# l646773422/h264-lab

Measured on AMD Instinct MI355X. Metric: 1080p macroblocks/sec, higher is better.
Workload: dtype u8

## Files before the change

### h264-lab_amd/csrc/h264e_host.c

```c
#include <stdio.h>
#include <stdlib.h>
#include <string.h>
#include <time.h>
#include <sched.h>
#include <pthread.h>
#include "../../include/h264e_mi355x.h"
#include "../../include/h264e_hip.h"

#define MAGIC 0x4D493335u
#define SLICE_P 0
#define SLICE_I 2

static int g_device = -1;
static __thread char g_host_err[256];

static int imin(int a, int b) { return a < b ? a : b; }
static int imax(int a, int b) { return a > b ? a : b; }

const char *H264E_last_error(void) { return g_host_err[0] ? g_host_err : h264e_hip_last_error(); }
void H264E_set_device(int device) { g_device = device; }
int H264E_device_count(void) { return h264e_hip_device_count(); }

static int pick_device(void)
{
// ... 723 lines not shown
        return H264E_STATUS_BAD_FRAME_TYPE;

    qp = rc_frame_start(&e->rc, e->param.gop, e->seq.nmb, e->param.vbv_size_bytes, opt->desired_frame_bytes,
                        e->run_param.qp_min, e->run_param.qp_max, key);

    memset(&task, 0, sizeof(task));
    task.active = 1; task.frame_index = 0;
    task.slice_type = key ? SLICE_I : SLICE_P;
    task.qp = qp; task.speed = opt->encode_speed;
    task.nslices = e->slices > 1 ? imin(e->slices, e->seq.nmby) : 1;
    slice_header_bits(&e->seq, key, e->frame_num, e->next_idr_pic_id, qp, e->pic_init_qp,
                      (opt->encode_speed == 8 || opt->encode_speed == 10), task.nslices, &task.hdr_nal, &task.hdr_bits, &task.hdr_nbits);
    build_qdat(task.qdat, qp, !key);

    memset(&res, 0, sizeof(res));
    den = e->denoise && opt->encode_speed < 2;
    if (den)
    {
        if (put_frame(m->pool, in, dev, win) || h264e_hip_denoise_frames(m->pool, 0, 1, !e->den_started)) return H264E_STATUS_BAD_ARGUMENT;
        e->den_started = 1;
        task.denoised = 1;
    }
    e->frames_in++;
    if (e->param.vbv_size_bytes && !key && e->rc.vbv_bits - opt->desired_frame_bytes*8 > e->param.vbv_size_bytes*8)
    {
        uint8_t rb[32];
        hbits_t b;
        size_t w;
        memset(&b, 0, sizeof(b));
        b.buf = rb;
        hb_put(&b, 8, (uint32_t)task.hdr_nal);
        hb_ue(&b, 0);
        hb_put(&b, task.hdr_nbits > 32 ? task.hdr_nbits - 32 : 0, (uint32_t)(task.hdr_nbits > 32 ? task.hdr_bits >> 32 : 0));
        hb_put(&b, task.hdr_nbits > 32 ? 32 : task.hdr_nbits, (uint32_t)task.hdr_bits);
        hb_ue(&b, (uint32_t)e->seq.nmb);
        hb_put(&b, 1, 1);
        if (b.n) hb_put(&b, 8 - b.n, 0);
        if (out_pos + 2*b.pos + 8 > cap) { snprintf(g_host_err, sizeof(g_host_err), "coded frame does not fit the scratch blob"); return H264E_STATUS_BAD_ARGUMENT; }
        w = nal_emit(out + out_pos, rb, b.pos);
        if (opt->nalu_callback) opt->nalu_callback(out + out_pos + 4, (int)(w - 4), opt->nalu_callback_token);
        out_pos += w;
        res.all_skipped = 1;
        if (!den && put_frame(m->pool, in, dev, win)) return H264E_STATUS_BAD_ARGUMENT;
    } else
    {
    if (!den && put_frame(m->pool, in, dev, win)) return H264E_STATUS_BAD_ARGUMENT;
    if (frame_exact(m->pool, &task, e->seq.nmbx, e->seq.nmby, e->clusters) || h264e_hip_stream_done(m->pool, 0, &res) != 1) return H264E_STATUS_BAD_ARGUMENT;
    {
        const uint8_t *nals = frame_nals(m->pool, 0, &res, m->rbsp, m->rbsp_cap);
        size_t w;
        if (!nals) return H264E_STATUS_BAD_ARGUMENT;
        w = emit_slices(out + out_pos, cap - out_pos, nals, &res, opt->nalu_callback, opt->nalu_callback_token);
        if (!w)
        {
            snprintf(g_host_err, sizeof(g_host_err), "coded frame does not fit the scratch blob");
            return H264E_STATUS_BAD_ARGUMENT;
        }
        out_pos += w;
    }
    }

    if (task.nslices == 1 || res.all_skipped) e->parent_all_skipped = res.all_skipped;
    rc_frame_end(&e->rc, e->seq.nmb, e->param.vbv_size_bytes, opt->desired_frame_bytes, (int)out_pos, key, e->parent_all_skipped);

    if (!e->param.const_input_flag && in)
    {
        int c, y;
        const uint8_t *s = m->recon;
        if (h264e_hip_read_recon(m->pool, 0, m->recon)) return H264E_STATUS_BAD_ARGUMENT;
        for (c = 0; c < 3; c++)
        {
            int w = e->seq.w >> (c ? 1 : 0), h = e->seq.h >> (c ? 1 : 0);
            for (y = 0; y < h; y++) memcpy(in->yuv[c] + (size_t)y*in->stride[c], s + (size_t)y*w, (size_t)w);
            s += (size_t)w*h;
        }
    }
    if (++e->frame_num >= e->param.gop && e->param.gop && e->run_param.frame_type == H264E_FRAME_TYPE_DEFAULT) e->frame_num = 0;
    e->have_recon = 1;
    *coded_data = out;
    *sizeof_coded_data = (int)out_pos;
    return H264E_STATUS_SUCCESS;
}

int H264E_encode(H264E_persist_t *p, H264E_scratch_t *scratch, const H264E_run_param_t *opt, H264E_io_yuv_t *in,
                 unsigned char **coded_data, int *sizeof_coded_data)
{
    return encode_frame(p, scratch, opt, in, NULL, NULL, coded_data, sizeof_coded_data);
}

int H264E_encode_device(H264E_persist_t *p, H264E_scratch_t *scratch, const H264E_run_param_t *opt, const H264E_dev_frame_t *frame,
                        unsigned char **coded_data, int *sizeof_coded_data)
{
    return encode_frame(p, scratch, opt, NULL, frame, NULL, coded_data, sizeof_coded_data);
}

int H264E_encode_device_scaled(H264E_persist_t *p, H264E_scratch_t *scratch, const H264E_run_param_t *opt, const H264E_dev_frame_t *frame,
                               const H264E_dev_window_t *win, unsigned char **coded_data, int *sizeof_coded_data)
{
    if (!frame || !win)
    {
        snprintf(g_host_err, sizeof(g_host_err), "H264E_encode_device_scaled: null %s", frame ? "window" : "frame");
        return H264E_STATUS_BAD_ARGUMENT;
    }
    return encode_frame(p, scratch, opt, NULL, frame, win, coded_data, sizeof_coded_data);
}

int H264E_read_recon_device(H264E_persist_t *p, const H264E_dev_frame_t *dst)
{
    henc_t *e = (henc_t *)p;
    impl_t mm;
    g_host_err[0] = 0;
    if (!impl_of(e, &mm)) return H264E_STATUS_BAD_ARGUMENT;
    if (!dst) { snprintf(g_host_err, sizeof(g_host_err), "H264E_read_recon_device: null destination"); return H264E_STATUS_BAD_ARGUMENT; }
    if (!e->have_recon)
    {
        snprintf(g_host_err, sizeof(g_host_err), "H264E_read_recon_device: no frame has been encoded yet");
        return H264E_STATUS_BAD_ARGUMENT;
    }
    return h264e_hip_egress_last(mm.pool, 0, dst->format, (void *const *)dst->plane, dst->stride, dst->pixel_bytes, dst->producer_stream) ? H264E_STATUS_BAD_ARGUMENT
                                                                                                                                     : H264E_STATUS_SUCCESS;
}

int H264E_read_quality(H264E_persist_t *p, uint64_t ssd[3], double ssim[3])
{
    henc_t *e = (henc_t *)p;
    impl_t mm;
    g_host_err[0] = 0;
    if (!impl_of(e, &mm)) return H264E_STATUS_BAD_ARGUMENT;
    if (!ssd && !ssim) { snprintf(g_host_err, sizeof(g_host_err), "H264E_read_quality: both outputs are NULL"); return H264E_STATUS_BAD_ARGUMENT; }
    if (!e->have_recon)
    {
        snprintf(g_host_err, sizeof(g_host_err), "H264E_read_quality: no frame has been encoded yet");
        return H264E_STATUS_BAD_ARGUMENT;
    }
    return h264e_hip_quality_last(mm.pool, 0, ssd, ssim) ? H264E_STATUS_BAD_ARGUMENT : H264E_STATUS_SUCCESS;
}

int H264E_ssim_planes(int device, const void *a, int a_stride, const void *b, int b_stride, int width, int height, double *ssim)
{
    h264e_hip_pool_t *pool = NULL;
    int rc;
    g_host_err[0] = 0;
    if (h264e_hip_pool_create(&pool, device < 0 ? pick_device() : device, 16, 16, 1, 1)) return -1;
    rc = h264e_hip_ssim_planes(pool, a, a_stride, b, b_stride, width, height, ssim);
    h264e_hip_pool_destroy(pool);
    return rc;
}

void *H264E_dev_malloc(int device, size_t bytes) { g_host_err[0] = 0; return h264e_hip_dev_malloc(device, bytes); }
void H264E_dev_free(void *p) { h264e_hip_dev_free(p); }
int H264E_dev_memcpy(void *dst, const void *src, size_t bytes, int to_device) { g_host_err[0] = 0; return h264e_hip_dev_memcpy(dst, src, bytes, to_device); }


#define CLIP_KEEP_MAX 8
typedef struct { int done, ring_lo, entries; } clip_pass_t;
struct H264E_clip_tag
{
    H264E_clip_param_t par;
    seq_t seq;
    int nframes, ring;
    int resident;
    int time_input;
    double input_ms;
    long long input_frames;
    h264e_hip_pool_t *pool;
    int next;
    int avail;
    int pending_avail;
    void (*idle_hook)(void *token); void *idle_token;
    int32_t state[2];
    int first_dev;
    int first_row;
    int32_t after[2]; int have_after;
    int narrow;
    int narrow_ok;
    int wide_until, wide_hold;
    int launch_base, launch_frames;
    int stopped_before;
    long long far_acc; int far_frames;
    int rc_on;
    rc_t rcs; int rc_frame, rc_qp;
    int rc_last_bytes[2];
    h264e_hip_mbrec_t **rec_store;
    int32_t (*used_store)[2];
    int32_t **permb_store;
    uint64_t *ssd_out;
    double *ssim_out;
    int recon_floor;
    int32_t *traj;
    uint8_t *big; size_t big_cap;
    h264e_hip_task_t *tasks;
    int32_t (*used)[2];
    clip_pass_t sc, la, den;
    int denoise, den_motion;
    struct clip_sched { uint8_t key, idr; int frame_num; } *sched;
    int *forced, nforced;
    int all_key;
    int scenecut;
    uint32_t *sc_hist;
    int *sc_dist; uint8_t *sc_cut;
    double sc_kernel_ms; long long sc_frames;
    uint8_t *qp_sched;
    int qp_explicit;
    int la_kbps, la_window, la_qmin, la_qmax;
    uint64_t *la_rec;
    int *la_bits;
    int la_planned, la_closed;
    uint64_t la_k[2];
    long long la_debt;
    double la_kernel_ms; long long la_frames;
    int la_search, la_any;
    int keep_on;
    int nkeep;
    struct clip_keep { int frame, rows, qp, nslices, speed, denoised; } keep[CLIP_KEEP_MAX];
};

static void clip_keep_drop(H264E_clip_t *c, int from)
{
    int i, k = 0;
    for (i = 0; i < c->nkeep; i++) if (c->keep[i].frame < from) c->keep[k++] = c->keep[i];
    c->nkeep = k;
}


static int clip_pass_pending(const H264E_clip_t *c, const clip_pass_t *p, const char *pass, int limit)
{
    if (limit - p->done > c->resident) { snprintf(g_host_err, sizeof(g_host_err), "%s: frames %d..%d do not fit the input ring", pass, p->done, limit - 1); return -1; }
    return imax(limit - p->done, 0);
}

static void clip_pass_made(clip_pass_t *p, int a, int limit)
{
    p->done = limit;
    p->ring_lo = imax(imin(p->ring_lo, a), limit - p->entries);
}

static int clip_pass_resident(const clip_pass_t *p, int frame, const char *who, const char *what)
{
    const int hi = p->done, lo = imin(p->ring_lo, hi);
    if (frame >= lo && frame < hi) return 1;
    if (lo < hi) snprintf(g_host_err, sizeof(g_host_err), "%s: frame %d has no %s on the device (frames %d..%d have)", who, frame, what, lo, hi - 1);
    else snprintf(g_host_err, sizeof(g_host_err), "%s: frame %d has no %s on the device (no frame has)", who, frame, what);
    return 0;
}

static void clip_inputs_replaced(H264E_clip_t *c, int first)
{
    if (first < c->sc.done) c->sc.done = first;
    if (first < c->la.done) c->la.done = first;
    if (first < c->den.done) c->den.done = first;
    clip_keep_drop(c, first);
}

static int clip_pass_predecessor_gone(const clip_pass_t *p, int first, const char *made, const char *kept, const char *ring)
{
    if (first <= 0 || first >= p->done || first - 1 >= p->done - p->entries) return 0;
    snprintf(g_host_err, sizeof(g_host_err), "upload: frame %d would be %s again, but the %s in front of it has left the %s (rewind and upload from frame 0)", first, made, kept, ring);
    return -1;
}

static void clip_sched_build(H264E_clip_t *c)
{
    const int gop = c->par.gop;
    int f, k = 0, fn = 0, parity = 0, all = 1;
    for (f = 0; f <= c->nframes; f++)
    {
        int forced, key;
        while (k < c->nforced && c->forced[k] < f) k++;
        forced = k < c->nforced && c->forced[k] == f;
        if (c->sc_cut && f < c->nframes)
        {
            c->sc_cut[f] = (uint8_t)(!forced && fn && c->scenecut && f < c->sc.done && c->sc_dist[f] > c->scenecut);
            forced |= c->sc_cut[f];
        }
        key = forced || fn == 0;
        if (key) { fn = 0; parity ^= 1; }
        c->sched[f].key = (uint8_t)key; c->sched[f].idr = (uint8_t)parity; c->sched[f].frame_num = fn;
        if (f < c->nframes) all &= key;
        if (++fn >= gop && gop && !forced) fn = 0;
    }
    c->all_key = all;
}

static int clip_nslices(const H264E_clip_t *c) { return c->par.slices > 1 ? imin(imin(c->par.slices, H264E_HIP_MAX_SLICES), c->seq.nmby) : 1; }

static void clip_launch_frames_reset(H264E_clip_t *c) { c->launch_frames = (c->par.slices > 1 || c->all_key) ? c->ring - 1 : c->launch_base; }

#define CLIP_DEV_BUDGET (24.0*1073741824.0)
static double clip_dev_slot_bytes(int nmb) { return (double)nmb*256.0*3.0 + (double)nmb*(64 + 96 + 8 + 640 + 660 + 2048 + 64) + 65536.0; }

int H264E_struct_size(int which) { return which == 0 ? (int)sizeof(H264E_clip_param_t) : which == 1 ? (int)sizeof(H264E_clip_stats_t) : which == 2 ? (int)sizeof(H264E_dev_frame_t) : -1; }

static double now_ms(void)
{
    struct timespec ts;
    clock_gettime(CLOCK_MONOTONIC, &ts);
    return ts.tv_sec*1e3 + ts.tv_nsec*1e-6;
}

#define LOOKAHEAD_K0_P 15086u
#define LOOKAHEAD_K0_KEY 14322u
#define LOOKAHEAD_K0_SEARCH 53818u

void H264E_clip_rewind(H264E_clip_t *c)
{
    if (!c) return;
    c->next = 0;
    c->state[0] = c->par.mv_clusters_in[0]; c->state[1] = c->par.mv_clusters_in[1];
    c->first_dev = 0;
    c->first_row = 0; c->have_after = 0; c->recon_floor = 0; c->stopped_before = 0;
    clip_keep_drop(c, 0);
    c->narrow = c->narrow_ok;
    c->wide_until = 0; c->wide_hold = 30; c->far_acc = 0; c->far_frames = 0;
    clip_launch_frames_reset(c);
    memset(&c->rcs, 0, sizeof(c->rcs));
    c->rc_frame = -1; c->rc_qp = c->par.qp; c->rc_last_bytes[0] = c->rc_last_bytes[1] = 0;
    c->la_planned = c->la_closed = 0; c->la_debt = 0;
    c->la_k[0] = c->la_search ? LOOKAHEAD_K0_SEARCH : LOOKAHEAD_K0_P; c->la_k[1] = LOOKAHEAD_K0_KEY;
}

int H264E_clip_open(H264E_clip_t **out, const H264E_clip_param_t *par, int nframes)
{
    H264E_clip_t *c;
    g_host_err[0] = 0;
    if (!out || !par || nframes <= 0 || par->width <= 0 || par->height <= 0 || ((par->width | par->height) & 1) || par->gop < 0) return -1;
    c = (H264E_clip_t *)calloc(1, sizeof(*c));
    if (!c) return -1;
    c->par = *par;
    c->rc_on = par->kbps > 0 || par->qp == 0;
    c->par.qp = imin(imax(par->qp, 10), 51);
    seq_init(&c->seq, par->width, par->height, par->vbv_size_bytes, 0);
    c->nframes = nframes;
    c->narrow_ok = (getenv("H264E_WIDE_WINDOW") || c->seq.nmb > 12000) ? 0 : 1;
    c->keep_on = getenv("H264E_KEEP_KEY_ROWS") ? atoi(getenv("H264E_KEEP_KEY_ROWS")) != 0 : 1;
    {
        const int nmb = c->seq.nmb;
        const int rows_budget = (par->slices > 1 || c->seq.nmby <= 135) ? 13000 : 6500;
        c->launch_base = par->max_chains > 0 ? par->max_chains : imax(imin(161, imax(13, rows_budget/imax(c->seq.nmby, 1) + 1)), imin(1025, 97*8160/imax(nmb, 1))) - 1;
        {
            const double host_slot = (double)nmb*168.0 + 65536.0 + 4096.0;
            const double dev_slot = clip_dev_slot_bytes(nmb);
            const double by_host = 896.0*1048576.0/host_slot, by_dev = CLIP_DEV_BUDGET/dev_slot;
            int cap = (int)(by_host < by_dev ? by_host : by_dev);
            cap = imin(imax(cap, c->launch_base), 1024);
            c->ring = (par->max_chains > 0 ? par->max_chains : cap) + 1;
        }
    }
    if (getenv("H264E_RING")) { c->ring = atoi(getenv("H264E_RING")); c->launch_base = imin(c->launch_base, imax(c->ring - 1, 1)); }
    c->ring = imax(2, imin(c->ring, nframes + 1));
    if (getenv("H264E_LAUNCH_BASE")) c->launch_base = atoi(getenv("H264E_LAUNCH_BASE"));
    c->launch_base = imax(1, imin(c->launch_base, c->ring - 1));
    c->resident = par->resident_frames > 0 ? imin(par->resident_frames, nframes) : nframes;
    c->den.entries = c->resident; c->la.entries = imax(c->resident, 2);
    c->traj = (int32_t *)malloc(sizeof(int32_t)*2*(size_t)c->seq.nmb);
    c->tasks = (h264e_hip_task_t *)calloc((size_t)c->ring, sizeof(*c->tasks));
    c->used = (int32_t (*)[2])calloc((size_t)c->ring, sizeof(int32_t[2]));
    c->sched = (struct clip_sched *)calloc((size_t)nframes + 1, sizeof(*c->sched));
    if (!c->traj || !c->tasks || !c->used || !c->sched) { free(c->traj); free(c->tasks); free(c->used); free(c->sched); free(c); return -1; }
    clip_sched_build(c);
    while (h264e_hip_pool_create(&c->pool, par->device, par->width, par->height, c->ring, c->resident))
    {
        if (c->ring <= c->launch_base + 1 || par->max_chains > 0)
        {
            free(c->traj); free(c->tasks); free(c->used); free(c->sched); free(c);
            return -1;
        }
        c->ring = imax(c->launch_base + 1, c->ring/2);
    }
    if (par->keep_records)
    {
        c->rec_store = (h264e_hip_mbrec_t **)calloc((size_t)nframes, sizeof(*c->rec_store));
        c->used_store = (int32_t (*)[2])calloc((size_t)nframes, sizeof(int32_t[2]));
        c->permb_store = (int32_t **)calloc((size_t)nframes, sizeof(*c->permb_store));
        if (!c->rec_store || !c->used_store || !c->permb_store) { H264E_clip_close(c); return -1; }
    }
    H264E_clip_rewind(c);
    *out = c;
    return 0;
}

void H264E_clip_close(H264E_clip_t *c)
{
    if (!c) return;
    h264e_hip_pool_destroy(c->pool);
    if (c->rec_store) { int f; for (f = 0; f < c->nframes; f++) { free(c->rec_store[f]); if (c->permb_store) free(c->permb_store[f]); } }
    free(c->rec_store); free(c->used_store); free(c->permb_store);
    free(c->traj); free(c->tasks); free(c->used); free(c->big);
    free(c->sched); free(c->forced); free(c->sc_hist); free(c->sc_dist); free(c->sc_cut);
    free(c->qp_sched); free(c->la_rec); free(c->la_bits);
    free(c);
}

static int clip_put_allowed(const H264E_clip_t *c, int first, int n)
{
    if (!c || first < 0 || n < 0 || first + n > c->nframes) { snprintf(g_host_err, sizeof(g_host_err), "upload: bad frame range"); return -1; }
    if (first + n - c->resident > c->next) { snprintf(g_host_err, sizeof(g_host_err), "upload: input ring full (frames %d.. are not encoded yet)", c->next); return -1; }
    if (c->denoise && clip_pass_predecessor_gone(&c->den, first, "denoised", "denoised picture", "input ring")) return -1;
    if ((c->la_kbps || c->den_motion) && clip_pass_predecessor_gone(&c->la, first, "analysed", "half-resolution picture", "ring")) return -1;
    return 0;
}

static int clip_ring_piece(const H264E_clip_t *c, int f, int n, int *run)
{
    *run = imin(n, c->resident - f % c->resident);
    return f % c->resident;
}

static int clip_put(H264E_clip_t *c, int first, int n, const uint8_t *i420, int async)
{
    size_t fsz;
    int done, slot, run;
    if (clip_put_allowed(c, first, n)) return -1;
    fsz = (size_t)c->seq.width*c->seq.height*3/2;
    for (done = 0; done < n; done += run)
    {
        slot = clip_ring_piece(c, first + done, n - done, &run);
        if (async ? h264e_hip_upload_i420_async(c->pool, slot, run, i420 + fsz*(size_t)done) : h264e_hip_upload_i420(c->pool, slot, run, i420 + fsz*(size_t)done))
        {
            g_host_err[0] = 0;
            return -1;
        }
    }
    if (async) { if (first + n > c->pending_avail) c->pending_avail = first + n; }
    else if (first + n > c->avail) c->avail = first + n;
    clip_inputs_replaced(c, first);
    return 0;
}

int H264E_clip_upload(H264E_clip_t *c, int first, int nframes, const uint8_t *i420)
{
    if (clip_put(c, first, nframes, i420, 0)) return -1;
    return h264e_hip_sync(c->pool);
}

static int clip_put_device(H264E_clip_t *c, int first, int nframes, const H264E_dev_frame_t *frames, const H264E_dev_window_t *win)
{
    int i, rc = 0;
    double ms = 0;
    for (i = 0; i < nframes; i++)
    {
        const H264E_dev_frame_t *f = &frames[i];
        if (win ? h264e_hip_scale_check(c->pool, (first + i) % c->resident, f->format, f->plane, f->stride, (const int *)win)
                : h264e_hip_ingest_check(c->pool, (first + i) % c->resident, f->format, f->plane, f->stride, f->pixel_bytes)) return -1;
    }
    if (c->time_input && h264e_hip_copy_timer_start(c->pool)) return -1;
    for (i = 0; i < nframes && !rc; i++)
    {
        const H264E_dev_frame_t *f = &frames[i];
        rc = win ? h264e_hip_scale_device_async(c->pool, (first + i) % c->resident, f->format, f->plane, f->stride, (const int *)win, f->producer_stream)
                 : h264e_hip_ingest_device_async(c->pool, (first + i) % c->resident, f->format, f->plane, f->stride, f->pixel_bytes, f->producer_stream);
    }
    if (c->time_input && !h264e_hip_copy_timer_stop(c->pool, &ms)) { c->input_ms += ms; c->input_frames += i; }
    if (h264e_hip_upload_wait(c->pool) || rc) return -1;
    if (first + nframes > c->avail) c->avail = first + nframes;
    clip_inputs_replaced(c, first);
    return 0;
}

int H264E_clip_upload_device(H264E_clip_t *c, int first, int nframes, const H264E_dev_frame_t *frames)
{
    g_host_err[0] = 0;
    if (clip_put_allowed(c, first, nframes)) return -1;
    if (!frames) { snprintf(g_host_err, sizeof(g_host_err), "upload_device: null argument"); return -1; }
    return clip_put_device(c, first, nframes, frames, NULL);
}

int H264E_clip_upload_device_scaled(H264E_clip_t *c, int first, int nframes, const H264E_dev_frame_t *frames, const H264E_dev_window_t *win)
{
    g_host_err[0] = 0;
    if (clip_put_allowed(c, first, nframes)) return -1;
    if (!frames || !win) { snprintf(g_host_err, sizeof(g_host_err), "upload_device_scaled: null %s", frames ? "window" : "frames"); return -1; }
    return clip_put_device(c, first, nframes, frames, win);
}

int H264E_clip_input_time(H264E_clip_t *c, int enable, double *kernel_ms, long long *frames)
{
    if (!c) return -1;
    c->time_input = enable != 0;
    if (kernel_ms) *kernel_ms = c->input_ms;
    if (frames) *frames = c->input_frames;
    return 0;
}

int H264E_clip_upload_async(H264E_clip_t *c, int first, int nframes, const uint8_t *pinned_i420) { return clip_put(c, first, nframes, pinned_i420, 1); }
int H264E_clip_upload_wait(H264E_clip_t *c)
{
    if (!c || h264e_hip_upload_wait(c->pool)) return -1;
    if (c->pending_avail > c->avail) c->avail = c->pending_avail;
    return 0;
}
int H264E_clip_upload_poll(H264E_clip_t *c)
{
    int busy;
    if (!c) return -1;
    busy = h264e_hip_upload_busy(c->pool);
    if (busy < 0) { g_host_err[0] = 0; return -1; }
    if (busy) return 0;
    if (c->pending_avail > c->avail) c->avail = c->pending_avail;
    return 1;
}
void H264E_clip_position(const H264E_clip_t *c, int *next_frame, int *uploaded_frames)
{
    if (next_frame) *next_frame = c ? c->next : 0;
    if (uploaded_frames) *uploaded_frames = c ? c->avail : 0;
}
void H264E_clip_set_idle_hook(H264E_clip_t *c, void (*hook)(void *token), void *token) { if (c) { c->idle_hook = hook; c->idle_token = token; } }
void *H264E_clip_host_alloc(size_t bytes) { return h264e_hip_host_alloc(bytes); }
void H264E_clip_host_free(void *p) { h264e_hip_host_free(p); }

int H264E_clip_generate_synth(H264E_clip_t *c, int first, int nframes, int t0, uint32_t seed)
{
    int done, slot, run;
    if (clip_put_allowed(c, first, nframes)) return -1;
    for (done = 0; done < nframes; done += run)
    {
        slot = clip_ring_piece(c, first + done, nframes - done, &run);
        if (h264e_hip_generate_synth(c->pool, slot, run, t0 + done, seed)) { g_host_err[0] = 0; return -1; }
    }
    if (first + nframes > c->avail) c->avail = first + nframes;
    clip_inputs_replaced(c, first);
    return h264e_hip_sync(c->pool);
// ... 416 lines not shown


static int clip_prepass_scenecut(H264E_clip_t *c, int limit)
{
    const int n = c->scenecut ? clip_pass_pending(c, &c->sc, "scenecut", limit) : 0, a = limit - n;
    float ms = 0;
    int f, b;
    if (n <= 0) return n;
    if (h264e_hip_scenecut_frames(c->pool, a % c->resident, n, c->sc_hist + (size_t)a*64, &ms)) return -1;
    for (f = a; f < limit; f++)
    {
        const uint32_t *h = c->sc_hist + (size_t)f*64;
        uint64_t sum = 0;
        for (b = 0; f && b < 64; b++) sum += h[b] > h[b - 64] ? h[b] - h[b - 64] : h[b - 64] - h[b];
        c->sc_dist[f] = (int)(sum*1024u/(2u*(uint64_t)c->seq.width*(uint64_t)c->seq.height));
    }
    c->sc_kernel_ms += ms; c->sc_frames += n;
    clip_pass_made(&c->sc, a, limit);
    clip_sched_build(c);
    return 0;
}

static int clip_prepass_lookahead(H264E_clip_t *c, int limit)
{
    const int n = clip_pass_pending(c, &c->la, "lookahead", limit), a = limit - n;
    float ms = 0;
    if (n <= 0) return n;
    if (c->la_search ? h264e_hip_lookahead_search_frames(c->pool, a, n, c->la_search, (unsigned long long *)(c->la_rec + 3*(size_t)a), &ms)
                     : h264e_hip_lookahead_frames(c->pool, a, n, (unsigned long long *)(c->la_rec + 3*(size_t)a), &ms)) return -1;
    c->la_kernel_ms += ms; c->la_frames += n;
    c->la_any = 1;
    clip_pass_made(&c->la, a, limit);
    return 0;
}

static int clip_prepass_denoise(H264E_clip_t *c, int limit)
{
    const int n = c->denoise && c->par.speed < 2 ? clip_pass_pending(c, &c->den, "denoise", limit) : 0, a = limit - n;
    if (n <= 0) return n;
    if (c->den_motion)
    {
        if (clip_prepass_lookahead(c, limit) || h264e_hip_mcdenoise_frames(c->pool, a, n, c->den_motion, a == 0)) return -1;
    }
    else if (h264e_hip_denoise_frames(c->pool, a % c->resident, n, a == 0)) return -1;
    clip_pass_made(&c->den, a, limit);
    return 0;
}

static int clip_la_header_bits(const H264E_clip_t *c, int key)
{
    uint8_t ps[128];
    return 40*clip_nslices(c) + (key ? 8*(int)write_sps_pps(&c->seq, 26, ps, NULL, NULL) : 0);
}

static uint64_t clip_la_texture_bits(uint64_t k, uint64_t cost, int q, int key)
{
    const unsigned __int128 v = ((unsigned __int128)k*cost*k_bits_per_mb[key][imin(q, 50) - 10]) >> 24;
    return v > LOOKAHEAD_BITS_MAX ? LOOKAHEAD_BITS_MAX : (uint64_t)v;
}

static void clip_la_plan_window(H264E_clip_t *c, int j)
{
    const int W = c->la_window, a = j*W, b = imin(a + W, c->nframes), dfb = c->la_kbps*1000/8/30;
    const long long T = 8LL*dfb*W, carry = c->la_debt > T/2 ? T/2 : c->la_debt < -(T/2) ? -(T/2) : c->la_debt, Tj = 8LL*dfb*(b - a) + carry;
    const int hk = clip_la_header_bits(c, 1), hp = clip_la_header_bits(c, 0);
    const int prev = j ? c->qp_sched[a - 1] : 0, qlo = prev ? imax(c->la_qmin, prev - LOOKAHEAD_QP_STEP) : c->la_qmin, qhi = prev ? imin(c->la_qmax, prev + LOOKAHEAD_QP_STEP) : c->la_qmax;
    int q, f;
    for (q = qlo; q < qhi; q++)
    {
        long long sum = 0;
        for (f = a; f < b; f++)
        {
            const int key = c->sched[f].key;
            sum += (key ? hk : hp) + (long long)clip_la_texture_bits(c->la_k[key], c->la_rec[3*(size_t)f + (key ? 0 : 1)], q, key);
        }
        if (sum <= Tj) break;
    }
    memset(c->qp_sched + a, q, (size_t)(b - a));
    c->la_planned = j + 1;
}

static void clip_la_close_window(H264E_clip_t *c, int j)
{
    const int W = c->la_window, a = j*W, b = imin(a + W, c->nframes), dfb = c->la_kbps*1000/8/30;
    const int hk = clip_la_header_bits(c, 1), hp = clip_la_header_bits(c, 0);
    long long actual = 0, num[2] = { 0, 0 };
    unsigned __int128 den[2] = { 0, 0 };
    int present[2] = { 0, 0 }, f, t;
    for (f = a; f < b; f++)
    {
        const int key = c->sched[f].key;
        actual += c->la_bits[f];
        num[key] += c->la_bits[f] - (key ? hk : hp);
        den[key] += (unsigned __int128)c->la_rec[3*(size_t)f + (key ? 0 : 1)]*k_bits_per_mb[key][imin(c->qp_sched[f], 50) - 10];
        present[key] = 1;
    }
    c->la_debt += 8LL*dfb*(b - a) - actual;
    for (t = 0; t < 2; t++)
        if (present[t] && den[t])
        {
            const uint64_t old = c->la_k[t], lo = old/4, hi = old*4 > LOOKAHEAD_K_MAX ? LOOKAHEAD_K_MAX : old*4;
            const unsigned __int128 kn = ((unsigned __int128)(num[t] > 0 ? num[t] : 0) << 24)/den[t];
            uint64_t k = kn > hi ? hi : (uint64_t)kn;
            if (k < lo) k = lo;
            c->la_k[t] = k ? k : 1;
        }
    c->la_closed = j + 1;
}

int H264E_clip_stamps(H264E_clip_t *c, unsigned long long *dst) { return c ? h264e_hip_stamps_read(c->pool, dst, 1) : -1; }


#define CLIP_RC_DEPTH_MAX 8
#define CLIP_HEDGE_MAX 32

typedef enum
{
    CLIP_GO_ON,
    CLIP_TAKE_LEAF,
    CLIP_STOP_LEAF_LOST, CLIP_STOP_MISSPEC, CLIP_STOP_QP_MISS, CLIP_STOP_QP_LEAF, CLIP_STOP_FULL,
    CLIP_RELAUNCH,
    CLIP_ERROR
} clip_step_t;
static const char *const k_clip_ended_by[CLIP_ERROR] = {
    [CLIP_GO_ON] = "all frames delivered",
    [CLIP_STOP_LEAF_LOST] = "the hedge leaf with the exact QP did not complete (its own mv_clusters validation, or stopped)",
    [CLIP_STOP_MISSPEC] = "mv_clusters mis-speculation",
    [CLIP_STOP_QP_MISS] = "QP miss, no hedge leaf with the exact QP",
    [CLIP_STOP_QP_LEAF] = "QP miss covered by a hedge leaf (nothing behind a leaf)",
    [CLIP_STOP_FULL] = "output buffer full",
    [CLIP_RELAUNCH] = "all frames delivered" };

typedef struct
{
    uint8_t *out; size_t cap, pos;
    int *frame_bytes;
    int first;
    int nslices, no_deblock, idr_state;
    int desired_frame_bytes, qp_min, qp_max, pic_init_qp;
    uint16_t qdat_i[2][42], qdat_p[2][42];
    int spin_retries;
    long long far_reads;
    int debug;
    H264E_clip_stats_t stats;
} clip_call_t;

typedef struct
{
    int n, limit;
    int F, nh;
    int qp_task[CLIP_RC_DEPTH_MAX];
    int hedge_level[CLIP_HEDGE_MAX], hedge_qp[CLIP_HEDGE_MAX];
    int kept_frames, kept_rows;
    int after_stop;
    double t_submit, t_first, t_last;
    double t_prev;
    int nvalid;
    int leaf;
    int moved_from, moved_to;
    clip_step_t step;
} clip_launch_t;

static int clip_end(H264E_clip_t *c, const clip_call_t *x, H264E_clip_stats_t *st, int rc)
{
    if (rc) { h264e_hip_release(c->pool); c->nkeep = 0; }
    if (st) *st = x->stats;
    return rc;
}

static clip_step_t clip_abort_launch(H264E_clip_t *c)
{
    (void)h264e_hip_stream_abort(c->pool);
    (void)h264e_hip_sync(c->pool);
    return CLIP_ERROR;
}

static int clip_qp_per_frame(const H264E_clip_t *c) { return c->qp_explicit || c->la_kbps; }

static int clip_pic_init_qp(const H264E_clip_t *c, const clip_call_t *x, int f)
{
    if (!clip_qp_per_frame(c)) return x->pic_init_qp;
    while (f > 0 && !c->sched[f].key) f--;
    return c->qp_sched[f];
}

static void clip_task_set_qp(const H264E_clip_t *c, const clip_call_t *x, h264e_hip_task_t *t, int f, int qp)
{
    const struct clip_sched *s = c->sched + f;
    t->qp = qp;
    if (c->rc_on || clip_qp_per_frame(c)) build_qdat(t->qdat, qp, !s->key);
    else memcpy(t->qdat, s->key ? x->qdat_i : x->qdat_p, sizeof(t->qdat));
    slice_header_bits(&c->seq, s->key, s->frame_num, x->idr_state ^ s->idr, qp, clip_pic_init_qp(c, x, f), x->no_deblock, x->nslices, &t->hdr_nal, &t->hdr_bits, &t->hdr_nbits);
}

static void clip_plan_launch(H264E_clip_t *c, const clip_call_t *x, clip_launch_t *l)
{
    const struct clip_sched *sched = c->sched;
    const int nmb = c->seq.nmb, K = c->ring, n = l->n, rc_on = c->rc_on;
    const int rc_depth = imax(1, imin(CLIP_RC_DEPTH_MAX, getenv("H264E_RC_DEPTH") ? atoi(getenv("H264E_RC_DEPTH")) : (nmb >= 60000 ? 3 : 6)));
    const int F = rc_on ? imax(1, imin(imin(K - 1, rc_depth), l->limit - n)) : imin(imin(K - 1, c->launch_frames), l->limit - n);
    h264e_hip_task_t *tasks = c->tasks;
    int32_t (*used)[2] = c->used;
    rc_t rc_ahead;
    int i, qp = c->rc_qp;
    memset(tasks, 0, sizeof(*tasks)*(size_t)K);
    if (rc_on && c->rc_frame != n)
    {
        qp = c->rc_qp = rc_frame_start(&c->rcs, c->par.gop, nmb, c->par.vbv_size_bytes, x->desired_frame_bytes, x->qp_min, x->qp_max, sched[n].key);
        c->rc_frame = n;
    }
    rc_ahead = c->rcs;
    for (i = 0; i < F; i++)
    {
        h264e_hip_task_t *t = tasks + i;
        const int f = n + i, key = sched[f].key;
        if (rc_on)
        {
            if (i > 0)
            {
                const int pkey = sched[f - 1].key, pred = c->rc_last_bytes[pkey] > 0 ? c->rc_last_bytes[pkey] : x->desired_frame_bytes;
                rc_frame_end(&rc_ahead, nmb, c->par.vbv_size_bytes, x->desired_frame_bytes, pred, pkey, 0);
                qp = rc_frame_start(&rc_ahead, c->par.gop, nmb, c->par.vbv_size_bytes, x->desired_frame_bytes, x->qp_min, x->qp_max, key);
            }
            l->qp_task[i] = qp;
        } else if (clip_qp_per_frame(c)) qp = c->qp_sched[f];
        t->active = 1; t->frame_index = f % c->resident;
        t->slice_type = key ? SLICE_I : SLICE_P;
        t->speed = c->par.speed;
        t->nslices = x->nslices;
        clip_task_set_qp(c, x, t, f, qp);
        t->stream_mode = 1; t->slot = f % K;
        t->ref_slot = key ? -1 : (f - 1) % K;
        t->ref_in_flight = !key && i > 0;
        t->mv_clusters[0] = used[i][0] = (i && c->have_after) ? c->after[0] : c->state[0];
        t->mv_clusters[1] = used[i][1] = (i && c->have_after) ? c->after[1] : c->state[1];
        t->walk_on_device = 1;
        t->exact_state[0] = c->state[0]; t->exact_state[1] = c->state[1];
        t->mv_clusters_per_mb = NULL;
        t->traj_from_device = (i == 0) && c->first_dev;
        t->first_row = (i == 0 && c->first_dev) ? c->first_row : 0;
        t->narrow_window = c->narrow;
        t->denoised = c->denoise && c->par.speed < 2;
    }
    l->nh = 0;
    if (rc_on && F > 1)
    {
        static const int dq[4] = { -1, 1, -2, 2 };
        const int rc_hedge = imax(0, imin(4, getenv("H264E_RC_HEDGE") ? atoi(getenv("H264E_RC_HEDGE")) : (nmb >= 60000 ? 0 : nmb >= 20000 ? 2 : 4)));
        int k, a;
        for (k = 1; k < F; k++)
            for (a = 0; a < rc_hedge; a++)
            {
                const int q = l->qp_task[k] + dq[a], j = F + l->nh;
                h264e_hip_task_t *t = tasks + j;
                if (q < x->qp_min || q > x->qp_max || l->nh >= CLIP_HEDGE_MAX || j + 2 >= K) continue;
                *t = tasks[k];
                clip_task_set_qp(c, x, t, n + k, q);
                t->slot = (n + j) % K;
                t->walk_parent = k;
                t->walk_quiet = 1;
                used[j][0] = used[k][0]; used[j][1] = used[k][1];
                l->hedge_level[l->nh] = k; l->hedge_qp[l->nh] = q; l->nh++;
            }
    }
    if (l->nh) c->recon_floor = n;
    l->kept_frames = l->kept_rows = 0;
    for (i = 0; i < c->nkeep && !l->nh; i++)
    {
        const struct clip_keep *k = c->keep + i;
        const int ti = k->frame - n;
        h264e_hip_task_t *t = tasks + imax(imin(ti, F - 1), 0);
        if (ti < 0 || ti >= F || !sched[k->frame].key || t->traj_from_device) continue;
        if (t->qp != k->qp || t->nslices != k->nslices || t->speed != k->speed || t->denoised != k->denoised) continue;
        t->first_row = k->rows;
        l->kept_frames++; l->kept_rows += k->rows;
    }
    c->nkeep = 0;
    l->F = F;
    l->after_stop = c->stopped_before;
    c->have_after = 0;
    l->t_first = l->t_last = l->t_prev = 0;
    l->nvalid = 0; l->leaf = l->moved_from = l->moved_to = -1;
    l->step = CLIP_GO_ON;
}

static int clip_wait_frame(H264E_clip_t *c, int slot, h264e_hip_result_t *r)
{
    int dn, idle = 0;
    memset(r, 0, sizeof(*r));
    while ((dn = h264e_hip_stream_done(c->pool, slot, r)) == 0)
    {
        if (!h264e_hip_busy(c->pool) && ++idle > 2) break;
        if (c->idle_hook) c->idle_hook(c->idle_token);
        sched_yield();
    }
    return dn ? dn : h264e_hip_stream_done(c->pool, slot, r);
}

static clip_step_t clip_frame_stopped(H264E_clip_t *c, clip_call_t *x, const clip_launch_t *l, int ti, int dn, const h264e_hip_result_t *r)
{
    if (dn < 0) return CLIP_ERROR;
    if (ti >= l->F) return h264e_hip_stream_abort(c->pool) ? CLIP_ERROR : CLIP_STOP_LEAF_LOST;
    if (dn == 2 && r->walk_status == 2)
    {
        c->first_row = r->first_bad/c->seq.nmbx;
        c->first_dev = 1;
        c->after[0] = r->state_out[0]; c->after[1] = r->state_out[1]; c->have_after = 1;
        x->stats.reencoded_gops++;
        return CLIP_STOP_MISSPEC;
    }
    if (h264e_hip_sync(c->pool) && strstr(h264e_hip_last_error(), "bounded spin expired") && x->spin_retries < 3)
    {
        x->spin_retries++;
        x->stats.spin_relaunches++;
        return CLIP_RELAUNCH;
    }
    if (!g_host_err[0] && !h264e_hip_last_error()[0]) snprintf(g_host_err, sizeof(g_host_err), "frame %d did not complete", l->n + ti);
    return CLIP_ERROR;
}

static clip_step_t clip_take_frame(H264E_clip_t *c, clip_call_t *x, clip_launch_t *l, int ti, const h264e_hip_result_t *r)
{
    const int nmb = c->seq.nmb, F = l->F, is_hedge = ti >= F;
    const int f = l->n + (is_hedge ? l->hedge_level[ti - F] : ti), key = c->sched[f].key, slot = c->tasks[ti].slot, per_mb = (ti == 0 && c->first_dev);
    const size_t start = x->pos, need = (key ? 64 : 0) + r->nbytes;
    const uint8_t *nals;
    const double t0 = now_ms();
    size_t w;
    int rc_miss = 0;
    l->leaf = -1;
    l->t_prev = l->t_last; l->t_last = t0;
    if (ti == 0) l->t_first = t0;
    if (r->overflow) { snprintf(g_host_err, sizeof(g_host_err), "bit buffer overflow (frame %d)", f); return clip_abort_launch(c); }
    if (r->in_device && c->big_cap < r->nbytes) { free(c->big); c->big_cap = (size_t)r->nbytes*2; c->big = (uint8_t *)malloc(c->big_cap); }
    nals = frame_nals(c->pool, slot, r, c->big, c->big_cap);
    if (!nals) { c->big_cap = 0; return clip_abort_launch(c); }
    if (x->pos + need > x->cap) return h264e_hip_stream_abort(c->pool) ? CLIP_ERROR : CLIP_STOP_FULL;
    if (key) x->pos += write_sps_pps(&c->seq, clip_pic_init_qp(c, x, f), x->out + x->pos, NULL, NULL);
    w = emit_slices(x->out + x->pos, x->cap - x->pos, nals, r, NULL, NULL);
    if (!w) { snprintf(g_host_err, sizeof(g_host_err), "malformed frame export"); return clip_abort_launch(c); }
    x->pos += w;
    if (x->frame_bytes) x->frame_bytes[f - x->first] = (int)(x->pos - start);
    if (c->la_kbps) c->la_bits[f] = 8*(int)(x->pos - start);
    if (c->rc_on)
    {
        rc_frame_end(&c->rcs, nmb, c->par.vbv_size_bytes, x->desired_frame_bytes, (int)(x->pos - start), key, r->all_skipped);
        c->rc_last_bytes[key] = (int)(x->pos - start);
        if (f + 1 < c->nframes && (!c->scenecut || f + 1 < c->sc.done))
        {
            const int qp = c->rc_qp = rc_frame_start(&c->rcs, c->par.gop, nmb, c->par.vbv_size_bytes, x->desired_frame_bytes, x->qp_min, x->qp_max, c->sched[f + 1].key);
            c->rc_frame = f + 1;
            if (is_hedge) rc_miss = 1;
            else if (ti + 1 < F && l->qp_task[ti + 1] != qp)
            {
                int hh;
                rc_miss = 1;
                for (hh = 0; hh < l->nh; hh++) if (l->hedge_level[hh] == ti + 1 && l->hedge_qp[hh] == qp) { l->leaf = F + hh; rc_miss = 0; }
            }
        } else if (is_hedge) rc_miss = 1;
    }
    if (c->rec_store)
    {
        const size_t rb = sizeof(h264e_hip_mbrec_t)*(size_t)nmb;
        if (!c->rec_store[f]) c->rec_store[f] = (h264e_hip_mbrec_t *)malloc(rb);
        if (!c->rec_store[f]) return CLIP_ERROR;
        memcpy(c->rec_store[f], h264e_hip_stream_mbrec(c->pool, slot), rb);
        c->used_store[f][0] = c->used[ti][0]; c->used_store[f][1] = c->used[ti][1];
        free(c->permb_store[f]); c->permb_store[f] = NULL;
        if (per_mb)
        {
            c->permb_store[f] = (int32_t *)malloc(sizeof(int32_t)*2*(size_t)nmb);
            if (!c->permb_store[f] || h264e_hip_stream_fetch_traj(c->pool, slot, 1, c->permb_store[f])) return CLIP_ERROR;
        }
    }
    c->state[0] = r->state_out[0]; c->state[1] = r->state_out[1];
    if (ti == 0) c->first_dev = 0;
    x->stats.assemble_ms += now_ms() - t0;
    l->nvalid++;
    x->far_reads += r->far_reads;
    if (x->debug) fprintf(stderr, "clip frame %d: %d far reads\n", f, r->far_reads);
    if (x->debug && key && ti > 0 && !is_hedge)
        fprintf(stderr, "clip key frame %d (task %d, first row %d): taken %.2f ms after the submit, %.2f ms after frame %d\n", f, ti, c->tasks[ti].first_row, t0 - l->t_submit, t0 - l->t_prev, f - 1);
    if (is_hedge) { l->moved_from = slot; l->moved_to = f % c->ring; }
    if (rc_miss)
    {
        if (h264e_hip_stream_abort(c->pool)) return CLIP_ERROR;
        x->stats.reencoded_gops++;
        return is_hedge ? CLIP_STOP_QP_LEAF : CLIP_STOP_QP_MISS;
    }
    return l->leaf >= 0 ? CLIP_TAKE_LEAF : CLIP_GO_ON;
}

static int clip_keep_collect(H264E_clip_t *c, const clip_launch_t *l)
{
    int ti;
    c->nkeep = 0;
    if (!c->keep_on || l->nh || (l->step != CLIP_STOP_MISSPEC && l->step != CLIP_STOP_FULL && l->step != CLIP_STOP_QP_MISS)) return 0;
    for (ti = l->nvalid; ti < l->F && c->nkeep < CLIP_KEEP_MAX; ti++)
    {
        const h264e_hip_task_t *t = c->tasks + ti;
        struct clip_keep *k = c->keep + c->nkeep;
        int rows = 0;
        if (t->slice_type != SLICE_I) continue;
        if (h264e_hip_stream_rows_complete(c->pool, t->slot, &rows)) return -1;
        if (rows <= 0) break;
        k->frame = l->n + ti; k->rows = rows; k->qp = t->qp; k->nslices = t->nslices; k->speed = t->speed; k->denoised = t->denoised;
        c->nkeep++;
    }
    return 0;
}

static int clip_settle(H264E_clip_t *c, clip_call_t *x, const clip_launch_t *l)
{
    const int K = c->ring, n = l->n, nvalid = l->nvalid;
    if (l->step == CLIP_RELAUNCH) (void)clip_abort_launch(c);
    else if (h264e_hip_sync(c->pool)) return -1;
    if (nvalid) x->spin_retries = 0;
    if (clip_keep_collect(c, l)) return -1;
    if (l->moved_from >= 0 && h264e_hip_stream_copy_picture(c->pool, l->moved_from, l->moved_to)) return -1;
    x->stats.encode_ms += now_ms() - l->t_submit;
    if (c->ssd_out && nvalid && h264e_hip_ssd_frames(c->pool, nvalid, n % c->resident, c->resident, n % K, K, c->ssd_out + 3*(size_t)(n - x->first))) return -1;
    if (c->ssim_out && nvalid && h264e_hip_ssim_frames(c->pool, nvalid, n % c->resident, c->resident, n % K, K, c->ssim_out + 3*(size_t)(n - x->first))) return -1;
    c->next = n + nvalid;
    if (l->after_stop && nvalid) { x->stats.relaunches_timed++; x->stats.first_frame_ms_after_relaunch += l->t_first - l->t_submit; }
    c->stopped_before = nvalid < l->F && l->step != CLIP_STOP_FULL;
    return 0;
}

static void clip_adapt(H264E_clip_t *c, const clip_call_t *x, const clip_launch_t *l)
{
    const int K = c->ring, nvalid = l->nvalid;
    if (nvalid < l->F && l->step != CLIP_STOP_FULL) c->launch_frames = imin(imax(c->launch_base, 2*nvalid), K - 1);
    else if (nvalid == l->F) c->launch_frames = imin(2*c->launch_frames, K - 1);
    if (c->narrow)
    {
        c->far_acc += x->far_reads; c->far_frames += nvalid;
        if (c->far_frames >= 8)
        {
            if (c->far_acc > (long long)c->far_frames*c->seq.nmb/8)
            {
                c->narrow = 0;
                c->wide_until = c->next + c->wide_hold;
                c->wide_hold = imin(c->wide_hold*2, 960);
            } else if (c->far_frames >= 64) c->wide_hold = 30;
            c->far_acc = 0; c->far_frames = 0;
        }
    } else if (c->narrow_ok && c->next >= c->wide_until) { c->narrow = 1; c->far_acc = 0; c->far_frames = 0; }
}

static void clip_debug_line(const H264E_clip_t *c, const clip_call_t *x, const clip_launch_t *l)
{
    const double t_end = now_ms();
    const int nvalid = l->nvalid;
    const double t_first = nvalid ? l->t_first : t_end, t_last = nvalid ? l->t_last : t_end;
    fprintf(stderr, "clip launch %d (first row %d, %s window, %lld far reads): %d frames in flight, %d valid, next %d; first frame after %.2f ms, then %.3f ms/frame, drained %.2f ms after the last, %d key rows kept in %d frames; ended by: %s%s\n",
            x->stats.rounds, c->tasks[0].first_row, c->tasks[0].narrow_window ? "narrow" : "wide", x->far_reads, l->F, nvalid, c->next, t_first - l->t_submit, nvalid > 1 ? (t_last - t_first)/(nvalid - 1 + (nvalid < l->F)) : 0.0, t_end - t_last, l->kept_rows, l->kept_frames,
            k_clip_ended_by[l->step], l->nh ? " (+ hedge leaves)" : "");
}

int H264E_clip_encode(H264E_clip_t *c, uint8_t *out, size_t cap, size_t *out_bytes, int *frame_bytes, int profile, H264E_clip_stats_t *st)
{
    clip_call_t x;
    clip_launch_t l;
    memset(&x, 0, sizeof(x));
    g_host_err[0] = 0;
    x.out = out; x.cap = cap; x.frame_bytes = frame_bytes; x.first = c->next;
    x.nslices = clip_nslices(c);
    x.no_deblock = (c->par.speed == 8 || c->par.speed == 10);
    x.idr_state = c->par.first_idr_pic_id_state & 1;
    x.desired_frame_bytes = c->par.kbps > 0 ? c->par.kbps*1000/8/30 : 0;
    x.qp_min = c->rc_on ? 10 : c->par.qp; x.qp_max = c->par.kbps > 0 ? 50 : c->rc_on ? 51 : c->par.qp;
    x.pic_init_qp = imax(imin(30, x.qp_max), x.qp_min);
    build_qdat(x.qdat_i, c->rc_qp, 0);
    build_qdat(x.qdat_p, c->rc_qp, 1);
    h264e_hip_profile(c->pool, profile);
    x.stats.chains = c->ring - 1;
    x.stats.first_frame = x.first;
    x.debug = getenv("H264E_DEBUG") != NULL;
    l.step = CLIP_GO_ON;

    while (c->next < c->avail && l.step != CLIP_STOP_FULL)
    {
        int ti = 0;
        l.n = c->next; l.limit = c->avail;
        if (clip_prepass_scenecut(c, l.limit)) return clip_end(c, &x, st, -1);
        if (c->la_kbps)
        {
            const int j = l.n/c->la_window, wend = imin((j + 1)*c->la_window, c->nframes);
            if (c->la_planned <= j)
            {
                if (c->avail < wend) break;
                if (clip_prepass_lookahead(c, l.limit)) return clip_end(c, &x, st, -1);
                clip_la_plan_window(c, j);
            }
            l.limit = wend;
        }
        clip_plan_launch(c, &x, &l);
        x.stats.rounds++;
        x.stats.kept_key_frames += l.kept_frames; x.stats.kept_key_rows += l.kept_rows;
        x.far_reads = 0;
        l.t_submit = now_ms();
        if (clip_prepass_denoise(c, l.limit) || h264e_hip_submit(c->pool, c->tasks)) return clip_end(c, &x, st, -1);
        do
        {
            h264e_hip_result_t r;
            const int dn = clip_wait_frame(c, c->tasks[ti].slot, &r);
            l.step = dn == 1 ? clip_take_frame(c, &x, &l, ti, &r) : clip_frame_stopped(c, &x, &l, ti, dn, &r);
            ti = l.step == CLIP_TAKE_LEAF ? l.leaf : ti + 1;
        } while (l.step == CLIP_TAKE_LEAF || (l.step == CLIP_GO_ON && ti < l.F));
        if (l.step == CLIP_ERROR || clip_settle(c, &x, &l)) return clip_end(c, &x, st, -1);
        clip_adapt(c, &x, &l);
        while (c->la_kbps && c->la_closed < c->la_planned && c->next >= imin((c->la_closed + 1)*c->la_window, c->nframes)) clip_la_close_window(c, c->la_closed);
        if (x.debug) clip_debug_line(c, &x, &l);
        if (l.step == CLIP_STOP_FULL && c->next == x.first)
        {
            snprintf(g_host_err, sizeof(g_host_err), "output buffer too small for one frame");
            return clip_end(c, &x, st, -1);
        }
    }
    x.stats.frames = c->next - x.first;
    x.stats.delivered_mbs = (long long)x.stats.frames*c->seq.nmb;
    {
        unsigned long long pm = 0;
        if (!h264e_hip_mb_counter(c->pool, &pm, 1)) x.stats.processed_mbs = (long long)pm;
    }
    x.stats.mv_clusters_out[0] = c->state[0]; x.stats.mv_clusters_out[1] = c->state[1];
    x.stats.next_idr_pic_id_state = c->next ? x.idr_state ^ c->sched[c->next - 1].idr : x.idr_state;
    h264e_hip_profile_read(c->pool, &x.stats.mb_kernel_ms, &x.stats.splice_kernel_ms, &x.stats.kernel_launches);
    if (out_bytes) *out_bytes = x.pos;
    return clip_end(c, &x, st, 0);
}



typedef struct
{
    H264E_clip_t *clip; h264e_hip_group_t *group;
    uint8_t *out; size_t cap; size_t *out_bytes; int *frame_bytes; H264E_clip_stats_t *st;
    int rc; char err[256];
} multi_arg_t;

static void *multi_thread(void *p)
{
    multi_arg_t *a = (multi_arg_t *)p;
    a->rc = H264E_clip_encode(a->clip, a->out, a->cap, a->out_bytes, a->frame_bytes, 0, a->st);
    if (a->rc) snprintf(a->err, sizeof(a->err), "%s", H264E_last_error());
    h264e_hip_group_leave(a->group, a->clip->pool);
    return NULL;
}

int H264E_clip_encode_multi(H264E_clip_t **clips, int nclips, uint8_t **out, const size_t *cap, size_t *out_bytes, int **frame_bytes, H264E_clip_stats_t *stats)
{
    multi_arg_t *a;
    pthread_t *th;
    int i, rc = 0, done = 0, saved_base[8] = { 0 };
    g_host_err[0] = 0;
    if (!clips || nclips <= 0 || nclips > 8 || !out || !cap || !out_bytes) { snprintf(g_host_err, sizeof(g_host_err), "clip_encode_multi: bad argument"); return -1; }
    for (i = 0; i < nclips; i++) if (!clips[i]) { snprintf(g_host_err, sizeof(g_host_err), "clip_encode_multi: clip %d is NULL", i); return -1; }
    if (nclips == 1) return H264E_clip_encode(clips[0], out[0], cap[0], &out_bytes[0], frame_bytes ? frame_bytes[0] : NULL, 0, stats);
    a = (multi_arg_t *)calloc((size_t)nclips, sizeof(*a));
    th = (pthread_t *)calloc((size_t)nclips, sizeof(*th));
    if (!a || !th) { free(a); free(th); snprintf(g_host_err, sizeof(g_host_err), "out of host memory"); return -1; }
    while (done < nclips && !rc)
    {
        h264e_hip_group_t *g = NULL;
        int first = done, n = 0, started = 0;
        if (h264e_hip_group_create(&g, clips[first]->par.device)) { snprintf(g_host_err, sizeof(g_host_err), "clip_encode_multi: %s", h264e_hip_last_error()); rc = -1; break; }
        while (first + n < nclips && !h264e_hip_group_join(g, clips[first + n]->pool)) n++;
        if (!n) { snprintf(g_host_err, sizeof(g_host_err), "clip_encode_multi: clip %d cannot join a launch group (%s)", first, h264e_hip_last_error()); h264e_hip_group_destroy(g); rc = -1; break; }
        for (i = first; i < first + n; i++)
        {
            saved_base[i] = clips[i]->launch_base;
            if (n > 1 && clips[i]->par.slices <= 1 && !clips[i]->all_key && !clips[i]->rc_on)
            {
                clips[i]->launch_base = imax(8, clips[i]->launch_base/3);
                clips[i]->launch_frames = imin(clips[i]->launch_frames, clips[i]->launch_base);
            }
            a[i].clip = clips[i]; a[i].group = g; a[i].out = out[i]; a[i].cap = cap[i]; a[i].out_bytes = &out_bytes[i];
            a[i].frame_bytes = frame_bytes ? frame_bytes[i] : NULL; a[i].st = stats ? &stats[i] : NULL;
            if (pthread_create(&th[i], NULL, multi_thread, &a[i])) { snprintf(g_host_err, sizeof(g_host_err), "clip_encode_multi: cannot start a thread"); rc = -1; break; }
            started++;
        }
        for (i = first + started; i < first + n; i++) h264e_hip_group_leave(g, clips[i]->pool);
        for (i = first; i < first + started; i++)
        {
            pthread_join(th[i], NULL);
            if (a[i].rc && !rc) { rc = a[i].rc; snprintf(g_host_err, sizeof(g_host_err), "clip %d: %s", i, a[i].err); }
        }
        for (i = first; i < first + n; i++) if (saved_base[i] > 0) clips[i]->launch_base = saved_base[i];
        h264e_hip_group_destroy(g);
        done = first + n;
    }
    free(a); free(th);
    return rc;
}
```

### h264-lab_amd/csrc/h264e_pool.h

```cpp
#ifndef H264E_POOL_H
#define H264E_POOL_H
#include "enc_denoise.h"
#include "enc_ingest.h"
#include "enc_egress.h"
#include "enc_scale.h"
#include "enc_scale_rgb.h"
#include "enc_hbd.h"
#include "enc_scenecut.h"
#include "enc_lookahead.h"
#include "enc_lookahead_search.h"
#include "enc_mcdenoise.h"
#include "enc_ssim.h"

static const h264e_color_t k_color_rows[4] = {
    { { 66, 129, 25 }, { -38, -74, 112 }, { 112, -94, -18 }, 16 },
    { { 77, 150, 29 }, { -43, -84, 127 }, { 127, -107, -20 }, 0 },
    { { 47, 157, 16 }, { -26, -86, 112 }, { 112, -102, -10 }, 16 },
    { { 54, 183, 19 }, { -29, -98, 127 }, { 127, -116, -11 }, 0 } };

static const h264e_icolor_t k_icolor_rows[4] = {
    { 298, 16, 409, -100, -208, 516 },
    { 256, 0, 359, -88, -183, 454 },
    { 298, 16, 459, -55, -136, 541 },
    { 256, 0, 403, -48, -120, 475 } };

static thread_local char g_err[256];
#define FAIL(...) do { snprintf(g_err, sizeof(g_err), __VA_ARGS__); return -1; } while (0)
extern "C" const char *h264e_hip_last_error(void) { return g_err; }


#define HIPCHK(x) do { hipError_t e_ = (x); if (e_ != hipSuccess) FAIL("%s: %s", #x, hipGetErrorString(e_)); } while (0)
static int dev_malloc(void **p, size_t n) { return hipMalloc(p, n ? n : 1) == hipSuccess ? 0 : -1; }
static void dev_free(void *p) { if (p) (void)hipFree(p); }

static int host_malloc(void **p, size_t n)
{
    if (hipHostMalloc(p, n ? n : 1, hipHostMallocMapped | hipHostMallocCoherent) != hipSuccess) return -1;
    memset(*p, 0, n ? n : 1);
    return 0;
}
static void host_free(void *p) { if (p) (void)hipHostFree(p); }

#define TASK_RING 128
static int imin_h(int a, int b) { return a < b ? a : b; }

#include <pthread.h>
#include <stdarg.h>
#define H264E_MAX_DEVICES 64
static pthread_mutex_t g_device_mu = PTHREAD_MUTEX_INITIALIZER;
static pthread_cond_t g_device_cv = PTHREAD_COND_INITIALIZER;
static int g_device_held[H264E_MAX_DEVICES];
static void device_token_take(int device)
{
    const unsigned d = (unsigned)device % H264E_MAX_DEVICES;
    pthread_mutex_lock(&g_device_mu);
    while (g_device_held[d]) pthread_cond_wait(&g_device_cv, &g_device_mu);
    g_device_held[d] = 1;
    pthread_mutex_unlock(&g_device_mu);
}
static void device_token_give(int device)
{
    const unsigned d = (unsigned)device % H264E_MAX_DEVICES;
    pthread_mutex_lock(&g_device_mu);
    g_device_held[d] = 0;
    pthread_cond_broadcast(&g_device_cv);
    pthread_mutex_unlock(&g_device_mu);
}

#include <errno.h>
#include <fcntl.h>
#include <sys/file.h>
#include <sys/stat.h>
#include <unistd.h>
static pthread_mutex_t g_guard_mu = PTHREAD_MUTEX_INITIALIZER;
static int g_guard_fd[H264E_MAX_DEVICES], g_guard_pools[H264E_MAX_DEVICES], g_guard_init;
static int process_guard_acquire(int device)
{
    const char *share = getenv("H264E_SHARE_DEVICE");
    int rc = 0;
    if ((share && atoi(share) == 1) || device < 0 || device >= H264E_MAX_DEVICES) return 0;
    pthread_mutex_lock(&g_guard_mu);
    if (!g_guard_init) { for (int i = 0; i < H264E_MAX_DEVICES; i++) g_guard_fd[i] = -1; g_guard_init = 1; }
    if (g_guard_pools[device]++ == 0)
    {
        char bus[64] = "", path[160];
        if (hipDeviceGetPCIBusId(bus, (int)sizeof(bus), device) != hipSuccess || !bus[0]) snprintf(bus, sizeof(bus), "dev%d", device);
        for (char *q = bus; *q; q++) if (*q == ':' || *q == '.' || *q == '/') *q = '_';
        snprintf(path, sizeof(path), "%s/h264e_mi355x_%s.lock", getenv("H264E_LOCK_DIR") ? getenv("H264E_LOCK_DIR") : "/tmp", bus);
        int fd = open(path, O_RDWR | O_CREAT | O_CLOEXEC | O_NOFOLLOW, 0666);
        if (fd >= 0) (void)fchmod(fd, 0666);
        if (fd < 0 && (errno == EACCES || errno == EPERM)) fd = open(path, O_RDONLY | O_CLOEXEC | O_NOFOLLOW);
        if (fd >= 0)
        {
            if (flock(fd, LOCK_EX | LOCK_NB))
            {
                char who[32] = "";
                const ssize_t n = read(fd, who, sizeof(who) - 1);
                if (n > 0) { who[n] = 0; for (char *q = who; *q; q++) if (*q == '\n') *q = 0; }
                snprintf(g_err, sizeof(g_err), "device %d (%s) is in use by another encoder process (pid %s): the macroblock kernel needs the device's wave slots to itself -- "
                         "give each process its own GPU, or encode several streams in ONE process (H264E_clip_encode_multi); H264E_SHARE_DEVICE=1 overrides", device, bus, who[0] ? who : "?");
                close(fd);
                g_guard_pools[device]--;
                rc = -1;
            } else
            {
                char me[32];
                const int n = snprintf(me, sizeof(me), "%ld\n", (long)getpid());
                if (ftruncate(fd, 0) == 0 && write(fd, me, (size_t)n) != n) {  }
                g_guard_fd[device] = fd;
            }
        } else if (errno == EACCES || errno == EPERM)
        {
            snprintf(g_err, sizeof(g_err), "device %d: lock file %.100s belongs to another user (their encoder owns the device); H264E_SHARE_DEVICE=1 overrides", device, path);
            g_guard_pools[device]--;
            rc = -1;
        } else if (errno != ENOENT && errno != ENOTDIR)
        {
            snprintf(g_err, sizeof(g_err), "device %d: cannot open lock file %.100s: %.40s (see H264E_LOCK_DIR, H264E_SHARE_DEVICE)", device, path, strerror(errno));
            g_guard_pools[device]--;
            rc = -1;
        }
    }
    pthread_mutex_unlock(&g_guard_mu);
    return rc;
}
static void process_guard_release(int device)
{
    if (device < 0 || device >= H264E_MAX_DEVICES) return;
    pthread_mutex_lock(&g_guard_mu);
    if (g_guard_init && g_guard_pools[device] > 0 && --g_guard_pools[device] == 0 && g_guard_fd[device] >= 0) { close(g_guard_fd[device]); g_guard_fd[device] = -1; }
    pthread_mutex_unlock(&g_guard_mu);
}

struct h264e_hip_group;
typedef struct h264e_hip_group h264e_hip_group_t;

struct h264e_hip_pool
{
    int device, nchains, frames_resident;
    h264e_geom_t G;
    size_t frame_bytes;
    uint8_t *clip;
    uint8_t *den;
    int den_frames, den_flip;
    hipEvent_t ev_copy;
    hipEvent_t ev_pass[2];
    int *sc_rec;
    uint8_t *la_lo;
    unsigned long long *la_rec;
    int la_entries; size_t la_entry_bytes;
    uint32_t *la_field;
    h264e_color_t cm;
    hipEvent_t ev_ingest[2];
    hipEvent_t ev_in[2];
    h264e_icolor_t icm;
    hipEvent_t ev_out[2];
    int out_timed; double out_ms; long long out_calls;
    uint8_t *qual_dev; size_t qual_doubles;
    hipEvent_t ev_q[2];
    int q_timed; double q_ssd_ms, q_ssim_ms; long long q_frames, q_ssd_frames;
    h264e_chain_dev_t *chains_host;
    h264e_chain_dev_t *chains_dev;
    h264e_frame_task_t *tasks_dev;
    h264e_frame_task_t *tasks_host;
    int *progress_all;
    int *errflag;
    unsigned long long *mb_counter;
    uint32_t *order;
    int *stepflags;
    uint32_t *order_host;
    int order_jobs, order_narrow, order_sliced;
    size_t order_count;
    h264e_hostdone_t *host_done;
    uint8_t **host_rbsp;
    h264e_hip_mbrec_t **host_mbrec;
    uint32_t host_rbsp_cap;
    int *abort_word;
    int *abort_dev;
    h264e_walkrec_t *walkrec;
    int32_t **traj_dev;
    int *traj_cur;
    unsigned long long *ssd_dev;
    uint8_t *heap; size_t heap_bytes;
    uint8_t *hheap; size_t hheap_bytes;
    int launch_counter;
    int holds_device;
    int *slot_launch;
    int32_t **clu_dev;
    int *ref_sel;
    int ring_pos, pending;
    int profile, prof_launches;
    int guarded;
    struct h264e_hip_group *group;
    int group_round;
    int waves;
    int test_upload_fail_at, async_uploads;
    int test_keep_rows_cap;
    double prof_mb_ms, prof_splice_ms;
    hipStream_t stream;
    hipStream_t copy_stream;
    hipStream_t abort_stream;
    hipEvent_t ev_t0, ev_t1, ev_prep;
    hipEvent_t ev[TASK_RING][3];
    int ev_pending;
    uint32_t *mcd_cells;
    hipEvent_t ev_mcd[2];
    int mcd_pending; double mcd_ms; long long mcd_frames;
};

typedef struct
{
    int jobs, narrow;
    int forced, all_intra;
    int sliced, parallel, tree;
} launch_shape_t;

#define H264E_GROUP_MAX 8
struct h264e_hip_group
{
    int device, nmembers, arrived, round, failed;
    struct
    {
        h264e_hip_pool_t *pool;
        h264e_frame_task_t *tasks;
        launch_shape_t shape;
        int pending;
    } member[H264E_GROUP_MAX];
    pthread_mutex_t mu;
    pthread_cond_t cv;
    hipStream_t stream;
    hipEvent_t ev_done, ev_t0[2], ev_t1[2];
    int timed[2];
    h264e_frame_task_t *tasks_dev; size_t tasks_cap;
    uint32_t *order_dev; size_t order_cap;
    int holds_device;
    char err[256];
};

extern "C" int h264e_hip_device_count(void)
{
    int n = 0;
    if (hipGetDeviceCount(&n) != hipSuccess) return 0;
    return n;
}

static void device_acquire(h264e_hip_pool_t *p)
{
    if (p->holds_device) return;
    device_token_take(p->device);
    p->holds_device = 1;
}
static void device_release(h264e_hip_pool_t *p)
{
    if (!p->holds_device) return;
    p->holds_device = 0;
    device_token_give(p->device);
}

extern "C" void h264e_hip_pool_destroy(h264e_hip_pool_t *p)
{
    if (!p) return;
    (void)hipSetDevice(p->device);
    if (p->stream) (void)hipStreamSynchronize(p->stream);
    if (p->copy_stream) (void)hipStreamSynchronize(p->copy_stream);
    if (p->abort_stream) (void)hipStreamSynchronize(p->abort_stream);
    device_release(p);
    host_free(p->hheap);
    free(p->host_rbsp); free(p->host_mbrec); free(p->slot_launch); free(p->order_host); free(p->tasks_host);
    dev_free(p->heap);
    dev_free(p->den);
    dev_free(p->sc_rec);
    dev_free(p->la_lo); dev_free(p->la_rec); dev_free(p->la_field); dev_free(p->mcd_cells);
    dev_free(p->qual_dev);
    if (p->stream)
    {
        (void)hipEventDestroy(p->ev_q[0]); (void)hipEventDestroy(p->ev_q[1]);
        for (int i = 0; i < TASK_RING; i++) for (int k = 0; k < 3; k++) (void)hipEventDestroy(p->ev[i][k]);
        (void)hipEventDestroy(p->ev_t0); (void)hipEventDestroy(p->ev_t1); (void)hipEventDestroy(p->ev_prep); (void)hipEventDestroy(p->ev_copy);
        (void)hipEventDestroy(p->ev_ingest[0]); (void)hipEventDestroy(p->ev_ingest[1]); (void)hipEventDestroy(p->ev_in[0]); (void)hipEventDestroy(p->ev_in[1]);
        (void)hipEventDestroy(p->ev_out[0]); (void)hipEventDestroy(p->ev_out[1]);
        (void)hipEventDestroy(p->ev_pass[0]); (void)hipEventDestroy(p->ev_pass[1]);
        (void)hipEventDestroy(p->ev_mcd[0]); (void)hipEventDestroy(p->ev_mcd[1]);
        (void)hipStreamDestroy(p->stream);
        if (p->copy_stream) (void)hipStreamDestroy(p->copy_stream);
        if (p->abort_stream) (void)hipStreamDestroy(p->abort_stream);
    }
    free(p->chains_host); free(p->clu_dev); free(p->ref_sel); free(p->traj_dev); free(p->traj_cur);
    if (p->guarded) process_guard_release(p->device);
    free(p);
}

#define H264E_ORDER_MAX_JOBS 65536
static int order_by_start_step(uint32_t *out, int rows, int lag, const int *member_jobs, int nmembers)
{
    int maxjobs = 0;
    for (int i = 0; i < nmembers; i++) if (member_jobs[i] > maxjobs) maxjobs = member_jobs[i];
    if (maxjobs < 1) return 0;
    const int maxkey = lag*(maxjobs - 1) + 2*(rows - 1);
    int *start = (int *)calloc((size_t)maxkey + 2, sizeof(int));
    if (!start) return -1;
    for (int i = 0; i < nmembers; i++) for (int j = 0; j < member_jobs[i]; j++) for (int r = 0; r < rows; r++) start[lag*j + 2*r + 1]++;
    for (int k = 0; k <= maxkey; k++) start[k + 1] += start[k];
    for (int j = 0; j < maxjobs; j++)
        for (int i = 0, base = 0; i < nmembers; base += member_jobs[i], i++)
            if (j < member_jobs[i])
                for (int r = 0; r < rows; r++) out[start[lag*j + 2*r]++] = ((uint32_t)(base + j) << 16) | (uint32_t)r;
    free(start);
    return 0;
}

static size_t order_capacity(const h264e_geom_t &G, int jobs) { return (size_t)jobs*(size_t)(8*((G.nmby + 7)/8 + 1)); }

static size_t order_into_bands(const h264e_geom_t &G, int jobs, const uint32_t *in, int total, uint32_t *out)
{
    const int bands = 8, per = (G.nmby + 7)/8 + 1;
    const size_t qlen = (size_t)per*jobs;
    uint32_t *q = (uint32_t *)malloc(sizeof(uint32_t)*8*qlen);
    int *fill = (int *)calloc((size_t)8*jobs, sizeof(int)), *want = (int *)calloc((size_t)8*jobs, sizeof(int));
    size_t cnt[8] = { 0 }, n = 0;
    if (!q || !fill || !want) { free(q); free(fill); free(want); return 0; }
    for (size_t i = 0; i < 8*qlen; i++) q[i] = H264E_ORDER_PAD;
    for (int i = 0; i < total; i++)
    {
        const int row = (int)(in[i] & 0xffffu), x = (row >= G.nmby ? bands - 1 : imin_h(bands - 1, row*bands/G.nmby)) & 7;
        want[8*(in[i] >> 16) + x]++;
    }
    for (int i = 0; i < total; i++)
    {
        const int row = (int)(in[i] & 0xffffu), jb = (int)(in[i] >> 16), x = (row >= G.nmby ? bands - 1 : imin_h(bands - 1, row*bands/G.nmby)) & 7;
        if (row == 0) for (int y = 0; y < 8; y++) if (!want[8*jb + y]) cnt[y] += (size_t)per;
        q[(size_t)x*qlen + cnt[x]++] = in[i];
        if (++fill[8*jb + x] == want[8*jb + x]) cnt[x] += (size_t)(per - want[8*jb + x]);
    }
    for (size_t k = 0; k < qlen; k++) for (int x = 0; x < 8; x++) out[n++] = q[(size_t)x*qlen + k];
    free(q); free(fill); free(want);
    return n;
}

static int build_order(h264e_hip_pool_t *p, int jobs, int narrow, int sliced, int bands)
{
    const h264e_geom_t &G = p->G;
    const int rows = G.nmby + 1, total = jobs*rows, lag = narrow ? H264E_NARROW_FRAME_LAG : H264E_FRAME_LAG;
    if (bands < 0) bands = getenv("H264E_XCD_BANDS") ? atoi(getenv("H264E_XCD_BANDS")) : (G.nmb >= 30000 && !sliced ? 8 : 0);
    if (bands != 0 && bands != 8) FAIL("dispatch order: %d XCD bands (H264E_XCD_BANDS): only 0 and 8 are supported", bands);
    uint32_t *tmp = bands ? (uint32_t *)malloc(sizeof(uint32_t)*(size_t)total) : p->order_host;
    int rc = tmp ? order_by_start_step(tmp, rows, lag, &jobs, 1) : -1;
    p->order_count = (size_t)total;
    if (!rc && bands && !(p->order_count = order_into_bands(G, jobs, tmp, total, p->order_host))) rc = -1;
    if (bands) free(tmp);
    if (rc) FAIL("out of host memory");
    return 0;
}

extern "C" int h264e_hip_pool_create(h264e_hip_pool_t **pool, int device, int width, int height, int nchains,
                                     int frames_resident)
{
    if (!pool || width <= 0 || height <= 0 || ((width | height) & 1) || nchains <= 0 || frames_resident <= 0)
        FAIL("h264e_hip_pool_create: bad argument");
    h264e_hip_pool_t *p = (h264e_hip_pool_t *)calloc(1, sizeof(*p));
    if (!p) FAIL("out of host memory");
    p->device = device; p->nchains = nchains; p->frames_resident = frames_resident;
    h264e_geom_t &G = p->G;
    G.width = width; G.height = height;
    G.nmbx = (width + 15) >> 4; G.nmby = (height + 15) >> 4; G.nmb = G.nmbx*G.nmby;
    G.W = G.nmbx*16; G.H = G.nmby*16;
    G.cropping = !!((width | height) & 15);
    G.lim_x0 = G.lim_y0 = -14*4;
    G.lim_x1 = (G.W - 2)*4; G.lim_y1 = (G.H - 2)*4;
    G.row_words = G.nmbx*(H264E_ROW_BYTES_PER_MB/4);
    const int knobs = getenv("H264E_TEST_KNOBS") && atoi(getenv("H264E_TEST_KNOBS")) == 1;
    G.spin_limit = 1u << 24;
    G.test_stall_row = -1;
    G.fz_wait_all = getenv("H264E_FZ_WAIT_ALL") ? atoi(getenv("H264E_FZ_WAIT_ALL")) : 0;
    p->test_upload_fail_at = -1;
    p->test_keep_rows_cap = -1;
    if (knobs)
    {
        if (getenv("H264E_TEST_KEEP_ROWS_CAP")) p->test_keep_rows_cap = atoi(getenv("H264E_TEST_KEEP_ROWS_CAP"));
        if (getenv("H264E_TEST_ROW_BYTES_PER_MB")) { const int b = atoi(getenv("H264E_TEST_ROW_BYTES_PER_MB"))/4; G.row_words = G.nmbx*(b > 1 ? b : 1); }
        if (getenv("H264E_TEST_SPIN_LIMIT")) G.spin_limit = (unsigned)atol(getenv("H264E_TEST_SPIN_LIMIT"));
        if (getenv("H264E_TEST_STALL_ROW")) G.test_stall_row = atoi(getenv("H264E_TEST_STALL_ROW"));
        if (getenv("H264E_TEST_UPLOAD_FAIL_AT")) p->test_upload_fail_at = atoi(getenv("H264E_TEST_UPLOAD_FAIL_AT"));
    }
    p->frame_bytes = (size_t)width*height*3/2;
    p->waves = getenv("H264E_WAVES") ? atoi(getenv("H264E_WAVES")) : 0;
    if (p->waves != 1 && p->waves != 2 && p->waves != 3 && p->waves != 4) p->waves = 0;
    int ndev = 0;
    if (hipGetDeviceCount(&ndev) != hipSuccess || ndev <= 0)
    {
        free(p);
        FAIL("no HIP device: the HIP path is mandatory (there is no CPU fallback)");
    }
    if (hipSetDevice(device) != hipSuccess) { free(p); FAIL("hipSetDevice(%d) failed", device); }
    {
        const int share = getenv("H264E_SHARE_DEVICE") && atoi(getenv("H264E_SHARE_DEVICE")) == 1;
        if (process_guard_acquire(device)) { free(p); return -1; }
        p->guarded = !share;
    }
    p->cm = k_color_rows[0]; p->icm = k_icolor_rows[0];
    if (hipStreamCreate(&p->stream) != hipSuccess || hipStreamCreate(&p->copy_stream) != hipSuccess || hipStreamCreate(&p->abort_stream) != hipSuccess) { if (p->guarded) process_guard_release(device); free(p); FAIL("hipStreamCreate failed"); }
    for (int i = 0; i < TASK_RING; i++) for (int k = 0; k < 3; k++) (void)hipEventCreate(&p->ev[i][k]);
    (void)hipEventCreate(&p->ev_t0); (void)hipEventCreate(&p->ev_t1); (void)hipEventCreate(&p->ev_prep); (void)hipEventCreate(&p->ev_copy);
    (void)hipEventCreate(&p->ev_ingest[0]); (void)hipEventCreate(&p->ev_ingest[1]); (void)hipEventCreate(&p->ev_in[0]); (void)hipEventCreate(&p->ev_in[1]);
    (void)hipEventCreate(&p->ev_out[0]); (void)hipEventCreate(&p->ev_out[1]);
    (void)hipEventCreate(&p->ev_pass[0]); (void)hipEventCreate(&p->ev_pass[1]);
    (void)hipEventCreate(&p->ev_mcd[0]); (void)hipEventCreate(&p->ev_mcd[1]);
    (void)hipEventCreate(&p->ev_q[0]); (void)hipEventCreate(&p->ev_q[1]);
    p->chains_host = (h264e_chain_dev_t *)calloc((size_t)nchains, sizeof(h264e_chain_dev_t));
    p->clu_dev = (int32_t **)calloc((size_t)nchains, sizeof(int32_t *));
    p->ref_sel = (int *)calloc((size_t)nchains, sizeof(int));
    p->traj_dev = (int32_t **)calloc((size_t)nchains, sizeof(int32_t *));
    p->traj_cur = (int *)calloc((size_t)nchains, sizeof(int));
    p->slot_launch = (int *)calloc((size_t)nchains, sizeof(int));
    p->host_rbsp = (uint8_t **)calloc((size_t)nchains, sizeof(uint8_t *));
    p->host_mbrec = (h264e_hip_mbrec_t **)calloc((size_t)nchains, sizeof(h264e_hip_mbrec_t *));
    p->tasks_host = (h264e_frame_task_t *)calloc((size_t)nchains, sizeof(h264e_frame_task_t));
    if (!p->chains_host || !p->clu_dev || !p->ref_sel || !p->traj_dev || !p->traj_cur || !p->slot_launch || !p->host_rbsp || !p->host_mbrec || !p->tasks_host)
    {
        h264e_hip_pool_destroy(p);
        FAIL("out of host memory");
    }
    int bad = 0;
    const size_t plane = (size_t)G.W*G.H*3/2;
    const uint32_t arena_cap = (uint32_t)((size_t)G.nmb*640 + 1024);
    const uint32_t nal_cap = (uint32_t)((size_t)G.nmb*660 + 4096);
    p->host_rbsp_cap = getenv("H264E_HOST_MIRROR_BYTES") ? (uint32_t)atol(getenv("H264E_HOST_MIRROR_BYTES")) : (uint32_t)((size_t)G.nmb*160 + 65536);
    if (p->host_rbsp_cap > nal_cap) p->host_rbsp_cap = nal_cap;
    for (int pass = 0; pass < 2 && !bad; pass++)
    {
        size_t pos = 0, hpos = 0;
        uint8_t *base = pass ? p->heap : 0, *hbase = pass ? p->hheap : 0;
        auto carve = [&](size_t n, size_t align) -> void * { pos = (pos + align - 1) & ~(align - 1); void *r = base ? base + pos : 0; pos += n ? n : 1; return r; };
        auto hcarve = [&](size_t n) -> void * { hpos = (hpos + 255) & ~(size_t)255; void *r = hbase ? hbase + hpos : 0; hpos += n; return r; };
        p->clip = (uint8_t *)carve(p->frame_bytes*(size_t)frames_resident, 4096);
        p->chains_dev = (h264e_chain_dev_t *)carve(sizeof(h264e_chain_dev_t)*(size_t)nchains, 256);
        p->tasks_dev = (h264e_frame_task_t *)carve(sizeof(h264e_frame_task_t)*(size_t)nchains*TASK_RING, 256);
        p->progress_all = (int *)carve(sizeof(int)*2*(size_t)nchains*G.nmby, 256);
        p->errflag = (int *)carve(sizeof(int), 256);
        p->mb_counter = (unsigned long long *)carve(sizeof(unsigned long long), 256);
        p->stepflags = (int *)carve(sizeof(int)*2*(size_t)nchains, 256);
        p->abort_dev = (int *)carve(64, 256);
        p->walkrec = (h264e_walkrec_t *)carve(sizeof(h264e_walkrec_t)*(size_t)nchains, 256);
        p->ssd_dev = (unsigned long long *)carve(sizeof(unsigned long long)*3*(size_t)nchains, 256);
        p->order = (uint32_t *)carve(sizeof(uint32_t)*order_capacity(G, nchains), 256);
        p->host_done = (h264e_hostdone_t *)hcarve(sizeof(h264e_hostdone_t)*(size_t)nchains);
        p->abort_word = (int *)hcarve(64);
        for (int c = 0; c < nchains; c++)
        {
            h264e_chain_dev_t &C = p->chains_host[c];
            uint8_t *rec = (uint8_t *)carve(2*plane, 4096);
            for (int k = 0; k < 2; k++)
            {
                C.rec[k][0] = rec + k*plane;
                C.rec[k][1] = C.rec[k][0] + (size_t)G.W*G.H;
                C.rec[k][2] = C.rec[k][1] + (size_t)G.W*G.H/4;
            }
            C.bottom = (h264e_mbbottom_t *)carve(sizeof(h264e_mbbottom_t)*(size_t)G.nmb, 256);
            C.pend = (h264e_mbpend_t *)carve(sizeof(h264e_mbpend_t)*(size_t)G.nmb, 256);
            C.progress = p->progress_all + (size_t)c*2*G.nmby;
            C.rowbits = (uint32_t *)carve(sizeof(uint32_t)*(size_t)G.nmby*G.row_words, 256);
            C.rowmeta = (h264e_rowmeta_t *)carve(sizeof(h264e_rowmeta_t)*(size_t)G.nmby, 256);
            C.mbrec = (h264e_mbrec_t *)carve(sizeof(h264e_mbrec_t)*(size_t)G.nmb, 256);
            C.arena = (uint8_t *)carve(arena_cap, 256);
            C.arena_cap = arena_cap;
            C.nal_arena = (uint8_t *)carve(nal_cap, 256);
            C.nal_cap = nal_cap;
            C.cursor = (uint32_t *)carve(16, 256);
            C.fout = (h264e_frameout_t *)carve(sizeof(h264e_frameout_t), 256);
            C.prof = (unsigned long long *)carve(sizeof(unsigned long long)*48, 256);
            C.far_reads = (int *)carve(sizeof(int)*(size_t)G.nmby, 256);
            p->clu_dev[c] = (int32_t *)carve(sizeof(int32_t)*2*(size_t)G.nmb, 256);
            p->traj_dev[c] = (int32_t *)carve(sizeof(int32_t)*4*(size_t)G.nmb, 256);
            p->host_rbsp[c] = (uint8_t *)hcarve(p->host_rbsp_cap + 64);
            p->host_mbrec[c] = (h264e_hip_mbrec_t *)hcarve(sizeof(h264e_hip_mbrec_t)*(size_t)G.nmb + 64);
        }
        if (!pass)
        {
            p->heap_bytes = pos + 4096; p->hheap_bytes = hpos + 4096;
            bad |= dev_malloc((void **)&p->heap, p->heap_bytes);
            bad |= host_malloc((void **)&p->hheap, p->hheap_bytes);
        }
    }
    if (bad)
    {
        h264e_hip_pool_destroy(p);
        FAIL("device allocation failed");
    }
    (void)hipMemset(p->heap, 0, p->heap_bytes);
    if (hipMemcpy(p->chains_dev, p->chains_host, sizeof(h264e_chain_dev_t)*(size_t)nchains, hipMemcpyHostToDevice) != hipSuccess)
    {
        h264e_hip_pool_destroy(p);
        FAIL("descriptor upload failed");
    }
    p->order_host = (uint32_t *)malloc(sizeof(uint32_t)*order_capacity(G, nchains));
    if (!p->order_host) { h264e_hip_pool_destroy(p); FAIL("out of host memory"); }
    p->order_jobs = -1;
    *pool = p;
    return 0;
}

extern "C" int h264e_hip_upload_i420(h264e_hip_pool_t *p, int first, int nframes, const uint8_t *host)
{
    if (!p || first < 0 || nframes < 0 || first + nframes > p->frames_resident) FAIL("upload_i420: bad range");
    HIPCHK(hipSetDevice(p->device));
    HIPCHK(hipMemcpyAsync(p->clip + p->frame_bytes*(size_t)first, host, p->frame_bytes*(size_t)nframes, hipMemcpyHostToDevice, p->stream));
    return 0;
}

extern "C" int h264e_hip_upload_i420_async(h264e_hip_pool_t *p, int first, int nframes, const uint8_t *host)
{
    if (!p || first < 0 || nframes < 0 || first + nframes > p->frames_resident) FAIL("upload_i420_async: bad range");
    if (p->async_uploads++ == p->test_upload_fail_at) FAIL("upload_i420_async: injected failure (H264E_TEST_UPLOAD_FAIL_AT)");
    HIPCHK(hipSetDevice(p->device));
    HIPCHK(hipMemcpyAsync(p->clip + p->frame_bytes*(size_t)first, host, p->frame_bytes*(size_t)nframes, hipMemcpyHostToDevice, p->copy_stream));
    return 0;
}

extern "C" int h264e_hip_upload_wait(h264e_hip_pool_t *p)
{
    if (!p) FAIL("upload_wait: null pool");
    HIPCHK(hipSetDevice(p->device));
    HIPCHK(hipStreamSynchronize(p->copy_stream));
    return 0;
}

extern "C" int h264e_hip_upload_busy(h264e_hip_pool_t *p)
{
    if (!p) return 0;
    (void)hipSetDevice(p->device);
    const hipError_t e = hipStreamQuery(p->copy_stream);
    if (e == hipErrorNotReady) return 1;
    if (e != hipSuccess) FAIL("upload: %s", hipGetErrorString(e));
    return 0;
}

extern "C" void *h264e_hip_host_alloc(size_t bytes)
{
    void *q = 0;
    return hipHostMalloc(&q, bytes ? bytes : 1, hipHostMallocDefault) == hipSuccess ? q : 0;
}

extern "C" void h264e_hip_host_free(void *q)
{
    if (q) (void)hipHostFree(q);
}


static int ssd_run(h264e_hip_pool_t *p, int n, int in0, int in_mod, const h264e_chain_dev_t *chains, int pic0, int pic_mod, uint64_t *out)
{
    const h264e_geom_t &G = p->G;
    HIPCHK(hipMemsetAsync(p->ssd_dev, 0, sizeof(unsigned long long)*3*(size_t)n, p->stream));
    if (p->q_timed) HIPCHK(hipEventRecord(p->ev_q[0], p->stream));
    bk_launch_ssd(n, (const uint8_t *)p->clip, p->frame_bytes, G.width, G.height, in0, in_mod, chains, pic0, pic_mod, G.W, p->ssd_dev, p->stream);
    HIPCHK(hipGetLastError());
    if (p->q_timed) HIPCHK(hipEventRecord(p->ev_q[1], p->stream));
    HIPCHK(hipMemcpyAsync(out, p->ssd_dev, sizeof(unsigned long long)*3*(size_t)n, hipMemcpyDeviceToHost, p->stream));
    HIPCHK(hipStreamSynchronize(p->stream));
    if (p->q_timed)
    {
        float f = 0;
        HIPCHK(hipEventElapsedTime(&f, p->ev_q[0], p->ev_q[1]));
        p->q_ssd_ms += f; p->q_ssd_frames += n;
    }
    return 0;
}

extern "C" int h264e_hip_ssd_frames(h264e_hip_pool_t *p, int n, int in0, int in_mod, int pic0, int pic_mod, uint64_t *out)
{
    if (!p || !out || n <= 0 || n > p->nchains || in_mod <= 0 || in_mod > p->frames_resident || pic_mod <= 0 || pic_mod > p->nchains) FAIL("ssd_frames: bad argument");
    HIPCHK(hipSetDevice(p->device));
    return ssd_run(p, n, in0, in_mod, (const h264e_chain_dev_t *)p->chains_dev, pic0, pic_mod, out);
}

static int wait_for_copy_stream(h264e_hip_pool_t *p)
{
    HIPCHK(hipEventRecord(p->ev_copy, p->copy_stream));
    HIPCHK(hipStreamWaitEvent(p->stream, p->ev_copy, 0));
    return 0;
}

static int ring_records_pieces(h264e_hip_pool_t *p, void *host, void *ring, size_t bytes, int E, int first, int n)
{
    for (int done = 0, run; done < n; done += run)
    {
        uint8_t *const entry = (uint8_t *)ring + bytes*(size_t)((first + done) % E);
        run = imin_h(n - done, E - (first + done) % E);
        if (!host) HIPCHK(hipMemsetAsync(entry, 0, bytes*(size_t)run, p->stream));
        else HIPCHK(hipMemcpyAsync((uint8_t *)host + bytes*(size_t)done, entry, bytes*(size_t)run, hipMemcpyDeviceToHost, p->stream));
    }
    return 0;
}
static int ring_records_zero(h264e_hip_pool_t *p, void *ring, size_t bytes, int E, int first, int n) { return ring_records_pieces(p, NULL, ring, bytes, E, first, n); }
static int ring_records_read(h264e_hip_pool_t *p, void *host, void *ring, size_t bytes, int E, int first, int n) { return ring_records_pieces(p, host, ring, bytes, E, first, n); }

static int la_nbx(const h264e_hip_pool_t *p) { return (p->G.width >> 1) >> 3; }
static int la_nby(const h264e_hip_pool_t *p) { return (p->G.height >> 1) >> 3; }


#ifdef H264E_EMU
static void bk_launch_denoise(const uint8_t *in, const uint8_t *prev, uint8_t *out, int width, int height, hipStream_t)
{
    for (int pl = 0; pl < 3; pl++)
    {
        const int w = width >> (pl ? 1 : 0), h = height >> (pl ? 1 : 0);
        const size_t off = pl ? (size_t)width*height + (pl == 2 ? (size_t)(width/2)*(height/2) : 0) : 0;
        const int aligned = !((((uintptr_t)in + off) | ((uintptr_t)prev + off) | ((uintptr_t)out + off) | (uintptr_t)w) & 3);
        for (int y = 0; y < h; y++)
            for (int g = 0; g < (w + 3)/4; g++) denoise_group(k_denoise_gain, in + off, prev + off, out + off, w, h, g, y, aligned);
    }
}
#endif

static int den_index(const h264e_hip_pool_t *p, int slot) { return p->frames_resident == 1 ? p->den_flip : slot; }
static uint8_t *den_frame(const h264e_hip_pool_t *p, int index) { return p->den + p->frame_bytes*(size_t)index; }

static int den_step(h264e_hip_pool_t *p, int s, int first_from_zero, int *prev)
{
    const int R = p->frames_resident;
    *prev = first_from_zero ? p->den_frames - 1 : R == 1 ? p->den_flip : (s + R - 1) % R;
    if (R == 1) p->den_flip ^= 1;
    return den_index(p, s);
}

extern "C" int h264e_hip_denoise_reset(h264e_hip_pool_t *p)
{
    if (!p) FAIL("denoise_reset: null pool");
    HIPCHK(hipSetDevice(p->device));
    if (!p->den)
    {
        p->den_frames = (p->frames_resident == 1 ? 2 : p->frames_resident) + 1;
        if (dev_malloc((void **)&p->den, p->frame_bytes*(size_t)p->den_frames)) { p->den = 0; FAIL("denoise: device allocation failed (%d frames)", p->den_frames); }
    }
    p->den_flip = 0;
    HIPCHK(hipMemsetAsync(p->den, 0, p->frame_bytes*(size_t)p->den_frames, p->stream));
    return 0;
}

extern "C" int h264e_hip_denoise_frames(h264e_hip_pool_t *p, int first, int n, int from_zero)
{
    const int R = p ? p->frames_resident : 0;
    if (!p || !p->den || first < 0 || first >= R || n < 0 || n > R) FAIL("denoise_frames: bad argument (or the denoiser is not on)");
    if (!n) return 0;
    HIPCHK(hipSetDevice(p->device));
    if (wait_for_copy_stream(p)) return -1;
    for (int i = 0; i < n; i++)
    {
        const int s = (first + i) % R;
        int prev;
        const int out = den_step(p, s, i == 0 && from_zero, &prev);
// ... 791 lines not shown
    if (!p || !a || !b || !out) FAIL("ssim_planes: null argument");
    if (w < SSIM_MIN_DIM || w > SSIM_MAX_DIM) FAIL("ssim_planes: width %d (%d to %d: one 8 x 8 window at least)", w, SSIM_MIN_DIM, SSIM_MAX_DIM);
    if (h < SSIM_MIN_DIM || h > SSIM_MAX_DIM) FAIL("ssim_planes: height %d (%d to %d: one 8 x 8 window at least)", h, SSIM_MIN_DIM, SSIM_MAX_DIM);
    if (a_stride < w) FAIL("ssim_planes: stride %d of plane a is below its %d row bytes", a_stride, w);
    if (b_stride < w) FAIL("ssim_planes: stride %d of plane b is below its %d row bytes", b_stride, w);
    HIPCHK(hipSetDevice(p->device));
#ifndef H264E_EMU
    if (!ingest_is_device_memory(p, a, (size_t)(h - 1)*(size_t)a_stride + (size_t)w))
        FAIL("ssim_planes: plane a (%p, %d rows %d bytes apart) is not memory of device %d, or not inside one allocation", a, h, a_stride, p->device);
    if (!ingest_is_device_memory(p, b, (size_t)(h - 1)*(size_t)b_stride + (size_t)w))
        FAIL("ssim_planes: plane b (%p, %d rows %d bytes apart) is not memory of device %d, or not inside one allocation", b, h, b_stride, p->device);
#endif
    memset(&A, 0, sizeof(A));
    A.a = (const uint8_t *)a; A.b = (const uint8_t *)b; A.a_stride = a_stride; A.b_stride = b_stride;
    A.width = w; A.height = h; A.W = w;
    A.max_tiles = ssim_max_tiles(w, h);
    if (qual_reserve(p, 1 + (size_t)A.max_tiles)) return -1;
    return ssim_run(p, A, 1, 1, out);
}

extern "C" int h264e_hip_quality_last(h264e_hip_pool_t *p, int chain, uint64_t ssd[3], double ssim[3])
{
    if (!p) FAIL("quality_last: null pool");
    if (chain < 0 || chain >= p->nchains) FAIL("quality_last: chain %d outside the pool's %d", chain, p->nchains);
    if (!ssd && !ssim) FAIL("quality_last: both outputs are NULL");
    if (ssim && (p->G.width < 2*SSIM_MIN_DIM || p->G.height < 2*SSIM_MIN_DIM))
        FAIL("quality_last: a %d x %d picture has a chroma plane without an 8 x 8 window: SSIM needs 16 x 16 at least", p->G.width, p->G.height);
    HIPCHK(hipSetDevice(p->device));
    if (qual_reserve(p, ssim ? 3*(1 + (size_t)ssim_max_tiles(p->G.width, p->G.height)) : 1)) return -1;
    h264e_chain_dev_t d = p->chains_host[chain];
    for (int pl = 0; pl < 3; pl++) d.rec[0][pl] = d.rec[p->ref_sel[chain]][pl];
    HIPCHK(hipStreamSynchronize(p->stream));
    HIPCHK(hipMemcpy(p->qual_dev, &d, sizeof(d), hipMemcpyHostToDevice));
    if (ssd && ssd_run(p, 1, 0, 1, (const h264e_chain_dev_t *)p->qual_dev, 0, 1, ssd)) return -1;
    if (ssim && ssim_frames_run(p, "quality_last", 1, 1, 0, 1, (const h264e_chain_dev_t *)p->qual_dev, 0, 1, ssim)) return -1;
    return 0;
}

extern "C" int h264e_hip_quality_time(h264e_hip_pool_t *p, int enable, double *ssd_ms, double *ssim_ms, long long *frames)
{
    if (!p) FAIL("quality_time: null pool");
    p->q_timed = enable != 0;
    if (ssd_ms) *ssd_ms = p->q_ssd_ms;
    if (ssim_ms) *ssim_ms = p->q_ssim_ms;
    if (frames) *frames = p->q_frames > p->q_ssd_frames ? p->q_frames : p->q_ssd_frames;
    return 0;
}

extern "C" void *h264e_hip_dev_malloc(int device, size_t bytes)
{
    void *q = 0;
    if (hipSetDevice(device) != hipSuccess) { snprintf(g_err, sizeof(g_err), "dev_malloc: hipSetDevice(%d) failed", device); return 0; }
    if (dev_malloc(&q, bytes)) { snprintf(g_err, sizeof(g_err), "dev_malloc: no %zu bytes on device %d", bytes, device); return 0; }
    return q;
}
extern "C" void h264e_hip_dev_free(void *q) { dev_free(q); }
extern "C" int h264e_hip_dev_memcpy(void *dst, const void *src, size_t bytes, int to_device)
{
    if (!dst || !src) FAIL("dev_memcpy: null argument");
    HIPCHK(hipMemcpy(dst, src, bytes, to_device ? hipMemcpyHostToDevice : hipMemcpyDeviceToHost));
    return 0;
}

extern "C" int h264e_hip_generate_synth(h264e_hip_pool_t *p, int first, int nframes, int t0, uint32_t seed)
{
    if (!p || first < 0 || nframes < 0 || first + nframes > p->frames_resident) FAIL("generate_synth: bad range");
    for (int i = 0; i < nframes; i++)
    {
        uint8_t *d = p->clip + p->frame_bytes*(size_t)(first + i);
        HIPCHK(hipSetDevice(p->device));
        bk_launch_synth(d, p->G.width, p->G.height, t0 + i, seed, p->stream);
    }
    HIPCHK(hipGetLastError());
    return 0;
}

extern "C" int h264e_hip_sync(h264e_hip_pool_t *p)
{
    if (!p) FAIL("sync: null pool");
    HIPCHK(hipSetDevice(p->device));
    if (p->group)
    {
        h264e_hip_group_t *g = p->group;
        const hipError_t eg = hipEventSynchronize(g->ev_done);
        pthread_mutex_lock(&g->mu);
        if (g->holds_device && !g->arrived) { g->holds_device = 0; device_token_give(g->device); }
        pthread_mutex_unlock(&g->mu);
        if (eg != hipSuccess) FAIL("group launch: %s", hipGetErrorString(eg));
        if (p->profile && g->nmembers && g->member[0].pool == p)
            for (int k = 0; k < 2; k++)
            {
                float a = 0;
                if (g->timed[k] && hipEventElapsedTime(&a, g->ev_t0[k], g->ev_t1[k]) == hipSuccess) { p->prof_mb_ms += a; p->prof_launches++; }
            }
    }
    {
        const hipError_t es = hipStreamSynchronize(p->stream);
        device_release(p);
        if (es != hipSuccess) FAIL("hipStreamSynchronize: %s", hipGetErrorString(es));
    }
    for (int i = 0; i < p->ev_pending; i++)
    {
        float a = 0, b = 0;
        HIPCHK(hipEventElapsedTime(&a, p->ev[i][0], p->ev[i][1]));
        HIPCHK(hipEventElapsedTime(&b, p->ev[i][1], p->ev[i][2]));
        p->prof_mb_ms += a; p->prof_splice_ms += b; p->prof_launches++;
    }
    p->ev_pending = 0;
    int err = 0;
    HIPCHK(hipMemcpy(&err, p->errflag, sizeof(int), hipMemcpyDeviceToHost));
    if (err)
    {
        (void)hipMemset(p->errflag, 0, sizeof(int));
        FAIL("macroblock kernel gave up waiting for the row above (bounded spin expired)");
    }
    device_release(p);
    p->pending = 0;
    return 0;
}

extern "C" void h264e_hip_release(h264e_hip_pool_t *p)
{
    if (!p) return;
    (void)hipSetDevice(p->device);
    if (p->stream) (void)hipStreamSynchronize(p->stream);
    device_release(p);
}


extern "C" int h264e_hip_group_create(h264e_hip_group_t **out, int device)
{
    if (!out) FAIL("group_create: null argument");
    h264e_hip_group_t *g = (h264e_hip_group_t *)calloc(1, sizeof(*g));
    if (!g) FAIL("out of host memory");
    g->device = device;
    pthread_mutex_init(&g->mu, 0); pthread_cond_init(&g->cv, 0);
    if (hipSetDevice(device) != hipSuccess || hipStreamCreate(&g->stream) != hipSuccess) { free(g); FAIL("group_create: no stream on device %d", device); }
    (void)hipEventCreate(&g->ev_done);
    for (int k = 0; k < 2; k++) { (void)hipEventCreate(&g->ev_t0[k]); (void)hipEventCreate(&g->ev_t1[k]); }
    *out = g;
    return 0;
}

#define H264E_RESIDENT_WG_V2 1536
#define H264E_RESIDENT_WG_V3 512
static int pick_variant(const launch_shape_t &s, int jobs, int nmby)
{
    if (s.forced) return s.forced;
    if (s.all_intra) return 0;
    if (jobs*nmby >= H264E_RESIDENT_WG_V2 && s.parallel && !s.tree) return 4;
    if (jobs*(nmby + 1) <= H264E_RESIDENT_WG_V3) return 3;
    return 2;
}

static hipError_t launch_mb(const h264e_geom_t &G, int narrow, int variant, int jobs, size_t nblocks, const h264e_frame_task_t *tasks, const uint32_t *order,
                            hipEvent_t before, hipEvent_t after, hipStream_t stream)
{
    hipError_t e = before ? hipEventRecord(before, stream) : hipSuccess;
    if (e != hipSuccess) return e;
    bk_launch_mb(G, narrow, variant, jobs, (unsigned)nblocks, tasks, order, stream);
    e = after ? hipEventRecord(after, stream) : hipSuccess;
    const hipError_t le = hipGetLastError();
    return le != hipSuccess ? le : e;
}

static int group_fail(h264e_hip_group_t *g, const char *fmt, ...)
{
    va_list ap;
    va_start(ap, fmt);
    vsnprintf(g->err, sizeof(g->err), fmt, ap);
    va_end(ap);
    return -1;
}

static int group_grow(h264e_hip_group_t *g, void **buf, size_t *cap, size_t need, size_t slack, size_t elem)
{
    if (need <= *cap) return 0;
    if (*buf) (void)hipFree(*buf);
    *cap = need + slack;
    if (hipMalloc(buf, elem**cap) == hipSuccess) return 0;
    *buf = 0; *cap = 0;
    return group_fail(g, "group launch: device allocation failed");
}

static int group_launch_geometry(h264e_hip_group_t *g, int narrow, h264e_frame_task_t *td, uint32_t *od)
{
    launch_shape_t m = { 0, narrow, 0, 1, 0, 0, 0 };
    int idx[H264E_GROUP_MAX], jobs[H264E_GROUP_MAX], n = 0, rc = 0;
    for (int k = 0; k < g->nmembers; k++)
        if (g->member[k].pending && g->member[k].shape.narrow == narrow)
        {
            const launch_shape_t &s = g->member[k].shape;
            idx[n] = k; jobs[n++] = s.jobs; m.jobs += s.jobs;
            if (s.forced) m.forced = s.forced;
            m.all_intra &= s.all_intra; m.parallel |= s.parallel; m.tree |= s.tree;
        }
    if (!n) return 0;
    m.parallel |= n >= 2;
    const h264e_geom_t &G = g->member[idx[0]].pool->G;
    const size_t total = (size_t)m.jobs*(size_t)(G.nmby + 1);
    if (m.jobs >= H264E_ORDER_MAX_JOBS) return group_fail(g, "group launch: too many jobs");
    h264e_frame_task_t *th = (h264e_frame_task_t *)malloc(sizeof(h264e_frame_task_t)*(size_t)m.jobs);
    uint32_t *oh = (uint32_t *)malloc(sizeof(uint32_t)*total);
    if (!th || !oh || order_by_start_step(oh, G.nmby + 1, narrow ? H264E_NARROW_FRAME_LAG : H264E_FRAME_LAG, jobs, n)) rc = group_fail(g, "out of host memory");
    for (int i = 0, b = 0; i < n && !rc; b += jobs[i++])
    {
        h264e_hip_pool_t *p = g->member[idx[i]].pool;
        memcpy(th + b, g->member[idx[i]].tasks, sizeof(h264e_frame_task_t)*(size_t)jobs[i]);
        if (hipEventRecord(p->ev_prep, p->stream) != hipSuccess || hipStreamWaitEvent(g->stream, p->ev_prep, 0) != hipSuccess) rc = group_fail(g, "group launch: cannot order the launch behind a member's stream");
    }
    if (!rc && (hipMemcpyAsync(td, th, sizeof(h264e_frame_task_t)*(size_t)m.jobs, hipMemcpyHostToDevice, g->stream) != hipSuccess ||
                hipMemcpyAsync(od, oh, sizeof(uint32_t)*total, hipMemcpyHostToDevice, g->stream) != hipSuccess)) rc = group_fail(g, "group launch: task upload failed");
    free(th); free(oh);
    if (!rc)
    {
        const hipError_t le = launch_mb(G, narrow, pick_variant(m, m.jobs, G.nmby), m.jobs, total, td, od, g->ev_t0[narrow], g->ev_t1[narrow], g->stream);
        if (le != hipSuccess) rc = group_fail(g, "group launch: %s", hipGetErrorString(le));
        else g->timed[narrow] = 1;
    }
    return rc ? rc : m.jobs;
}

static int group_launch_locked(h264e_hip_group_t *g)
{
    const size_t rows = (size_t)g->member[0].pool->G.nmby + 1;
    size_t need_tasks = 0, off = 0;
    int rc = 0;
    g->err[0] = 0;
    g->timed[0] = g->timed[1] = 0;
    for (int k = 0; k < g->nmembers; k++) if (g->member[k].pending) need_tasks += (size_t)g->member[k].shape.jobs;
    if (hipSetDevice(g->device) != hipSuccess) rc = group_fail(g, "group launch: hipSetDevice(%d) failed", g->device);
    if (!rc) rc = group_grow(g, (void **)&g->tasks_dev, &g->tasks_cap, need_tasks, 64, sizeof(h264e_frame_task_t));
    if (!rc) rc = group_grow(g, (void **)&g->order_dev, &g->order_cap, need_tasks*rows, 4096, sizeof(uint32_t));
    if (!rc && need_tasks && !g->holds_device) { device_token_take(g->device); g->holds_device = 1; }
    for (int narrow = 0; narrow < 2 && !rc; narrow++)
    {
        const int jobs = group_launch_geometry(g, narrow, g->tasks_dev + off, g->order_dev + off*rows);
        if (jobs < 0) rc = -1; else off += (size_t)jobs;
    }
    if (hipEventRecord(g->ev_done, g->stream) != hipSuccess && !rc) rc = group_fail(g, "group launch: hipEventRecord failed");
    if (rc && !g->err[0]) (void)group_fail(g, "group launch failed");
    if (rc) snprintf(g_err, sizeof(g_err), "%s", g->err);
    for (int k = 0; k < g->nmembers; k++) { free(g->member[k].tasks); g->member[k].tasks = 0; g->member[k].pending = 0; }
    g->arrived = 0;
    g->failed = rc;
    g->round++;
    pthread_cond_broadcast(&g->cv);
    return rc;
}

static int group_submit(h264e_hip_pool_t *p, const h264e_frame_task_t *host, const launch_shape_t &s)
{
    h264e_hip_group_t *g = p->group;
    int rc = 0, k;
    pthread_mutex_lock(&g->mu);
    for (k = 0; k < g->nmembers && g->member[k].pool != p; k++) ;
    if (k == g->nmembers) { pthread_mutex_unlock(&g->mu); FAIL("group_submit: not a member"); }
    g->member[k].tasks = (h264e_frame_task_t *)malloc(sizeof(h264e_frame_task_t)*(size_t)s.jobs);
    if (!g->member[k].tasks) { pthread_mutex_unlock(&g->mu); FAIL("out of host memory"); }
    memcpy(g->member[k].tasks, host, sizeof(h264e_frame_task_t)*(size_t)s.jobs);
    g->member[k].shape = s; g->member[k].pending = 1;
    p->group_round = g->round;
    g->arrived++;
    if (g->arrived == g->nmembers) rc = group_launch_locked(g);
    else
    {
        const int r = g->round;
        while (g->round == r) pthread_cond_wait(&g->cv, &g->mu);
        rc = g->failed;
    }
    if (rc) snprintf(g_err, sizeof(g_err), "%s", g->err[0] ? g->err : "group launch failed");
    pthread_mutex_unlock(&g->mu);
    return rc;
}

extern "C" int h264e_hip_group_join(h264e_hip_group_t *g, h264e_hip_pool_t *p)
{
    if (!g || !p || p->group) FAIL("group_join: bad argument");
    pthread_mutex_lock(&g->mu);
    const int window = (12 - H264E_NARROW_FRAME_LAG)*(p->G.nmby + 1)/2, room = 1400/(window > 0 ? window : 1);
    int bad = g->nmembers >= H264E_GROUP_MAX || (g->nmembers >= 1 && g->nmembers >= room) || p->device != g->device || g->arrived;
    if (!bad && g->nmembers)
    {
        const h264e_geom_t &A = g->member[0].pool->G, &B = p->G;
        bad = A.width != B.width || A.height != B.height || A.row_words != B.row_words || A.spin_limit != B.spin_limit;
    }
    if (!bad) { memset(&g->member[g->nmembers], 0, sizeof(g->member[0])); g->member[g->nmembers++].pool = p; p->group = g; }
    pthread_mutex_unlock(&g->mu);
    if (bad) FAIL("group_join: the group is full (at most %d streams of this picture size share a launch), busy, on another device or holds another picture size", room < H264E_GROUP_MAX ? room : H264E_GROUP_MAX);
    return 0;
}

extern "C" void h264e_hip_group_leave(h264e_hip_group_t *g, h264e_hip_pool_t *p)
{
    if (!g || !p || p->group != g) return;
    pthread_mutex_lock(&g->mu);
    int k;
    for (k = 0; k < g->nmembers && g->member[k].pool != p; k++) ;
    if (k < g->nmembers)
    {
        if (g->member[k].pending) { free(g->member[k].tasks); g->arrived--; }
        memmove(&g->member[k], &g->member[k + 1], sizeof(g->member[0])*(size_t)(g->nmembers - 1 - k));
        g->nmembers--;
        if (g->nmembers && g->arrived == g->nmembers) (void)group_launch_locked(g);
        if (!g->nmembers && g->holds_device)
        {
            (void)hipSetDevice(g->device);
            (void)hipStreamSynchronize(g->stream);
            g->holds_device = 0; device_token_give(g->device);
        }
    }
    p->group = 0;
    pthread_mutex_unlock(&g->mu);
}

extern "C" void h264e_hip_group_destroy(h264e_hip_group_t *g)
{
    if (!g) return;
    (void)hipSetDevice(g->device);
    (void)hipStreamSynchronize(g->stream);
    for (int k = 0; k < g->nmembers; k++) { g->member[k].pool->group = 0; if (g->member[k].pending) free(g->member[k].tasks); }
    if (g->tasks_dev) (void)hipFree(g->tasks_dev);
    if (g->order_dev) (void)hipFree(g->order_dev);
    if (g->holds_device) { g->holds_device = 0; device_token_give(g->device); }
    (void)hipEventDestroy(g->ev_done);
    for (int k = 0; k < 2; k++) { (void)hipEventDestroy(g->ev_t0[k]); (void)hipEventDestroy(g->ev_t1[k]); }
    (void)hipStreamDestroy(g->stream);
    pthread_mutex_destroy(&g->mu); pthread_cond_destroy(&g->cv);
    free(g);
}


static int submit_check(const h264e_hip_pool_t *p, const h264e_hip_task_t *tasks, launch_shape_t *s)
{
    const h264e_geom_t &G = p->G;
    int any_narrow = 0, any_wide = 0, max_slices = 1;
    memset(s, 0, sizeof(*s));
    s->forced = p->waves; s->all_intra = 1;
    for (int c = 0; c < p->nchains; c++)
    {
        const h264e_hip_task_t &t = tasks[c];
        if (!t.active) continue;
        if (t.frame_index < 0 || t.frame_index >= p->frames_resident ||
            t.qp < 10 || t.qp > 51 || t.hdr_nbits < 0 || t.hdr_nbits > 56 || t.nslices < 0 || t.nslices > H264E_MAX_SLICES || t.nslices > G.nmby)
            FAIL("submit: bad task for chain %d", c);
        if (t.denoised && !p->den) FAIL("submit: task %d asks for the denoised picture, but the denoiser is not on", c);
        if (t.stream_mode && (t.slot < 0 || t.slot >= p->nchains || t.ref_slot >= p->nchains || (t.slice_type == 0 && t.ref_slot < 0) ||
                              (t.ref_in_flight && t.ref_slot < 0)))
            FAIL("submit: bad stream task %d", c);
        s->jobs = c + 1;
        if (t.slice_type != 2) s->all_intra = 0;
        if (t.nslices > max_slices) max_slices = t.nslices;
        if (t.stream_mode && t.walk_quiet) s->tree = 1;
        if (t.stream_mode && t.narrow_window) any_narrow = 1; else any_wide = 1;
    }
    if (any_narrow && any_wide) FAIL("submit: the jobs of one launch must agree on narrow_window");
    if (s->jobs >= H264E_ORDER_MAX_JOBS) FAIL("submit: too many jobs");
    s->narrow = any_narrow;
    s->sliced = max_slices >= 2;
    s->parallel = s->sliced || G.nmby >= 200;
    return 0;
}

static void fill_pictures(h264e_hip_pool_t *p, const h264e_hip_task_t *tasks, int c, h264e_frame_task_t &d)
{
    const h264e_hip_task_t &t = tasks[c];
    if (!t.stream_mode)
    {
        const int rs = p->ref_sel[c];
        d.chain = c;
        for (int k = 0; k < 3; k++) { d.ref[k] = p->chains_host[c].rec[rs][k]; d.dec[k] = p->chains_host[c].rec[rs ^ 1][k]; }
        p->ref_sel[c] ^= 1;
        return;
    }
    d.chain = t.slot;
    d.abort_word = p->abort_dev;
    if (t.walk_on_device)
    {
        const int par = t.walk_parent > 0 ? t.walk_parent - 1 : c - 1;
        d.walk_on_device = 1;
        d.walk_quiet = t.walk_quiet;
        d.exact_state[0] = t.exact_state[0]; d.exact_state[1] = t.exact_state[1];
        d.walk_out = p->walkrec + t.slot;
        d.walk_prev = (par >= 0 && par < c && tasks[par].active && tasks[par].stream_mode && tasks[par].walk_on_device) ? p->walkrec + tasks[par].slot : 0;
        d.traj_out = p->traj_dev[t.slot] + (size_t)(p->traj_cur[t.slot] ^ 1)*2*p->G.nmb;
    }
    for (int k = 0; k < 3; k++)
    {
        d.dec[k] = p->chains_host[t.slot].rec[0][k];
        d.ref[k] = t.ref_slot >= 0 ? p->chains_host[t.ref_slot].rec[0][k] : p->chains_host[t.slot].rec[1][k];
    }
    d.dep_progress = t.ref_in_flight ? p->chains_host[t.ref_slot].progress : 0;
}

static void fill_slice_rows(const h264e_geom_t &G, int nslices, h264e_frame_task_t &d)
{
    int mby = 0;
    d.nslices = nslices > 1 ? nslices : 1;
    for (int k = 0; k < d.nslices; k++) { d.slice_row[k] = (int16_t)mby; mby += (G.nmby - mby)/(d.nslices - k); }
    d.slice_row[d.nslices] = (int16_t)G.nmby;
}

static int fill_clusters(h264e_hip_pool_t *p, const h264e_hip_task_t &t, int c, h264e_frame_task_t &d)
{
    const size_t n = sizeof(int32_t)*2*(size_t)p->G.nmb;
    const int cs = t.stream_mode ? t.slot : c;
    d.clusters[0] = t.mv_clusters[0]; d.clusters[1] = t.mv_clusters[1];
    if (t.stream_mode && t.traj_from_device) d.clusters_per_mb = p->traj_dev[t.slot] + (size_t)p->traj_cur[t.slot]*2*p->G.nmb;
    else if (t.mv_clusters_per_mb)
    {
        if (hipStreamSynchronize(p->stream) != hipSuccess || hipMemcpy(p->clu_dev[cs], t.mv_clusters_per_mb, n, hipMemcpyHostToDevice) != hipSuccess) FAIL("mv_clusters upload failed");
        d.clusters_per_mb = p->clu_dev[cs];
    }
    return 0;
}

static int fill_task(h264e_hip_pool_t *p, const h264e_hip_task_t *tasks, int c, int launch_id, h264e_frame_task_t &d)
{
    const h264e_geom_t &G = p->G;
    const h264e_hip_task_t &t = tasks[c];
    const uint8_t *f = t.denoised ? den_frame(p, den_index(p, t.frame_index)) : p->clip + p->frame_bytes*(size_t)t.frame_index;
    d.active = t.active;
    d.in[0] = f; d.in[1] = f + (size_t)G.width*G.height; d.in[2] = d.in[1] + (size_t)(G.width/2)*(G.height/2);
    d.in_stride[0] = G.width; d.in_stride[1] = d.in_stride[2] = G.width/2;
    d.slice_type = t.slice_type; d.qp = t.qp; d.speed = t.speed;
    d.no_deblock = (t.speed == 8 || t.speed == 10);
    fill_pictures(p, tasks, c, d);
    d.arena_reset = 1;
    d.stepflags = p->stepflags + 2*c;
    d.host_done = p->host_done + d.chain;
    d.host_rbsp = p->host_rbsp[d.chain]; d.host_rbsp_cap = p->host_rbsp_cap;
    d.host_mbrec = (h264e_mbrec_t *)p->host_mbrec[d.chain];
    d.chain_desc = p->chains_dev + d.chain;
    d.errflag = p->errflag;
    d.mb_counter = p->mb_counter;
    d.first_row = (t.stream_mode && t.first_row > 0 && t.first_row <= G.nmby) ? t.first_row : 0;
    d.narrow = t.stream_mode && t.narrow_window;
    d.hdr_nal = t.hdr_nal; d.hdr_nbits = t.hdr_nbits; d.hdr_bits = t.hdr_bits;
    fill_slice_rows(G, t.nslices, d);
    if (fill_clusters(p, t, c, d)) return -1;
    memcpy(d.qdat, t.qdat, sizeof(d.qdat));
    d.launch_id = launch_id;
    p->host_done[d.chain].done = 0;
    p->slot_launch[d.chain] = launch_id;
    if (d.walk_on_device) p->traj_cur[t.slot] ^= 1;
    return 0;
}

static int reset_progress(h264e_hip_pool_t *p, const h264e_frame_task_t *host)
{
    const h264e_geom_t &G = p->G;
    hipError_t e = hipMemsetAsync(p->progress_all, 0, sizeof(int)*2*(size_t)p->nchains*G.nmby, p->stream);
    for (int c = 0; c < p->nchains && e == hipSuccess; c++)
        if (host[c].active && host[c].first_row > 0)
        {
            int *done = (int *)malloc(sizeof(int)*(size_t)host[c].first_row), *progress = p->chains_host[host[c].chain].progress;
            if (!done) { e = hipErrorOutOfMemory; break; }
            for (int r = 0; r < host[c].first_row; r++) done[r] = G.nmbx + 1;
            e = hipMemcpyAsync(progress, done, sizeof(int)*(size_t)host[c].first_row, hipMemcpyHostToDevice, p->stream);
            if (e == hipSuccess) e = hipMemcpyAsync(progress + G.nmby, done, sizeof(int)*(size_t)host[c].first_row, hipMemcpyHostToDevice, p->stream);
            free(done);
        }
    if (e != hipSuccess) FAIL("progress reset: %s", hipGetErrorString(e));
    return 0;
}

static int solo_launch(h264e_hip_pool_t *p, const h264e_frame_task_t *slot, const launch_shape_t &s)
{
    const int pe = p->ev_pending;
    if (s.jobs != p->order_jobs || s.narrow != p->order_narrow || s.sliced != p->order_sliced)
    {
        if (build_order(p, s.jobs, s.narrow, s.sliced, -1)) return -1;
        HIPCHK(hipMemcpyAsync(p->order, p->order_host, sizeof(uint32_t)*p->order_count, hipMemcpyHostToDevice, p->stream));
        p->order_jobs = s.jobs; p->order_narrow = s.narrow; p->order_sliced = s.sliced;
    }
    const hipError_t e = launch_mb(p->G, s.narrow, pick_variant(s, s.jobs, p->G.nmby), s.jobs, p->order_count, slot, p->order,
                                   p->profile ? p->ev[pe][0] : 0, p->profile ? p->ev[pe][1] : 0, p->stream);
    if (e != hipSuccess) FAIL("macroblock kernel launch: %s", hipGetErrorString(e));
    if (p->profile)
    {
        HIPCHK(hipEventRecord(p->ev[pe][2], p->stream));
        p->ev_pending++;
    }
    return 0;
}

extern "C" int h264e_hip_submit(h264e_hip_pool_t *p, const h264e_hip_task_t *tasks)
{
    launch_shape_t s;
    if (!p || !tasks) FAIL("submit: null argument");
    HIPCHK(hipSetDevice(p->device));
    if (submit_check(p, tasks, &s)) return -1;
    if (!s.jobs) return 0;
    if (p->pending >= TASK_RING - 1 && h264e_hip_sync(p)) return -1;
    h264e_frame_task_t *host = p->tasks_host;
    const int launch_id = ++p->launch_counter;
    memset(host, 0, sizeof(h264e_frame_task_t)*(size_t)p->nchains);
    for (int c = 0; c < p->nchains; c++)
        if (tasks[c].active && fill_task(p, tasks, c, launch_id, host[c])) return -1;
    if (!p->group) device_acquire(p);
    h264e_frame_task_t *slot = p->tasks_dev + (size_t)p->ring_pos*p->nchains;
    p->ring_pos = (p->ring_pos + 1) % TASK_RING;
    p->pending++;
    const hipError_t e = hipMemcpyAsync(slot, host, sizeof(h264e_frame_task_t)*(size_t)p->nchains, hipMemcpyHostToDevice, p->stream);
    if (e != hipSuccess) FAIL("task upload: %s", hipGetErrorString(e));
    if (reset_progress(p, host)) return -1;
    return p->group ? group_submit(p, host, s) : solo_launch(p, slot, s);
}


extern "C" int h264e_hip_stream_done(h264e_hip_pool_t *p, int slot, h264e_hip_result_t *res)
{
    if (!p || slot < 0 || slot >= p->nchains) FAIL("stream_done: bad argument");
    const volatile h264e_hostdone_t *d = p->host_done + slot;
    const int v = d->done;
    if (v != p->slot_launch[slot] && v != -p->slot_launch[slot]) return 0;
    __atomic_thread_fence(__ATOMIC_ACQUIRE);
    if (res)
    {
        res->walk_status = d->walk_status; res->first_bad = d->first_bad; res->state_out[0] = d->state_out[0]; res->state_out[1] = d->state_out[1];
        if (v > 0)
        {
            res->nbytes = d->nbytes; res->all_skipped = d->all_skipped; res->clusters_moved = d->clusters_moved; res->overflow = d->overflow; res->far_reads = d->far_reads;
            res->nslices = d->nslices; res->in_device = d->in_device;
            for (int k = 0; k < H264E_HIP_MAX_SLICES; k++) res->slice_nbytes[k] = d->slice_nbytes[k];
        }
    }
    return v > 0 ? 1 : 2;
}

extern "C" int h264e_hip_stream_rows_complete(h264e_hip_pool_t *p, int slot, int *rows)
{
    if (!p || !rows || slot < 0 || slot >= p->nchains) FAIL("stream_rows_complete: bad argument");
    const h264e_geom_t &G = p->G;
    int n = 0;
    if (p->slot_launch[slot] == p->launch_counter && ((const volatile h264e_hostdone_t *)p->host_done)[slot].done == p->launch_counter) n = G.nmby;
    else
    {
        int *host = (int *)malloc(sizeof(int)*(size_t)G.nmby);
        if (!host) FAIL("out of host memory");
        (void)hipSetDevice(p->device);
        hipError_t e = hipMemcpyAsync(host, p->chains_host[slot].progress, sizeof(int)*(size_t)G.nmby, hipMemcpyDeviceToHost, p->stream);
        if (e == hipSuccess) e = hipStreamSynchronize(p->stream);
        while (e == hipSuccess && n < G.nmby && host[n] == G.nmbx + 1) n++;
        free(host);
        if (e != hipSuccess) FAIL("stream_rows_complete: %s", hipGetErrorString(e));
    }
    if (p->test_keep_rows_cap >= 0 && n > p->test_keep_rows_cap) n = p->test_keep_rows_cap;
    *rows = n;
    return 0;
}

extern "C" int h264e_hip_stream_fetch_traj(h264e_hip_pool_t *p, int slot, int consumed, int32_t *dst)
{
    if (!p || !dst || slot < 0 || slot >= p->nchains) FAIL("stream_fetch_traj: bad argument");
    const int32_t *src = p->traj_dev[slot] + (size_t)(p->traj_cur[slot] ^ (consumed ? 1 : 0))*2*p->G.nmb;
    HIPCHK(hipSetDevice(p->device));
    HIPCHK(hipMemcpy(dst, src, sizeof(int32_t)*2*(size_t)p->G.nmb, hipMemcpyDeviceToHost));
    return 0;
}

extern "C" int h264e_hip_stream_copy_picture(h264e_hip_pool_t *p, int from, int to)
{
    if (!p || from < 0 || to < 0 || from >= p->nchains || to >= p->nchains) FAIL("stream_copy_picture: bad argument");
    if (from == to) return 0;
    const size_t plane = (size_t)p->G.W*p->G.H*3/2;
    HIPCHK(hipSetDevice(p->device));
    HIPCHK(hipMemcpyAsync(p->chains_host[to].rec[0][0], p->chains_host[from].rec[0][0], plane, hipMemcpyDeviceToDevice, p->stream));
    HIPCHK(hipStreamSynchronize(p->stream));
    return 0;
}

extern "C" const uint8_t *h264e_hip_stream_rbsp(h264e_hip_pool_t *p, int slot)
{
    return (p && slot >= 0 && slot < p->nchains) ? p->host_rbsp[slot] : 0;
}

extern "C" int h264e_hip_stream_fetch_nals(h264e_hip_pool_t *p, int slot, uint8_t *dst, uint32_t nbytes)
{
    if (!p || !dst || slot < 0 || slot >= p->nchains || nbytes > p->chains_host[slot].nal_cap) FAIL("stream_fetch_nals: bad argument");
    HIPCHK(hipSetDevice(p->device));
    HIPCHK(hipMemcpyAsync(dst, p->chains_host[slot].nal_arena, nbytes, hipMemcpyDeviceToHost, p->copy_stream));
    HIPCHK(hipStreamSynchronize(p->copy_stream));
    return 0;
}

extern "C" int h264e_hip_download_i420(h264e_hip_pool_t *p, int first, int nframes, uint8_t *host)
{
    if (!p || !host || first < 0 || nframes < 0 || first + nframes > p->frames_resident) FAIL("download_i420: bad range");
    HIPCHK(hipSetDevice(p->device));
    HIPCHK(hipMemcpy(host, p->clip + p->frame_bytes*(size_t)first, p->frame_bytes*(size_t)nframes, hipMemcpyDeviceToHost));
    return 0;
}

extern "C" const h264e_hip_mbrec_t *h264e_hip_stream_mbrec(h264e_hip_pool_t *p, int slot)
{
    return (p && slot >= 0 && slot < p->nchains) ? p->host_mbrec[slot] : 0;
}

extern "C" int h264e_hip_stream_abort(h264e_hip_pool_t *p)
{
    if (!p || !p->abort_word) FAIL("stream_abort: bad argument");
    __atomic_store_n(p->abort_word, p->launch_counter, __ATOMIC_RELEASE);
    HIPCHK(hipSetDevice(p->device));
    HIPCHK(hipMemsetD32Async((hipDeviceptr_t)p->abort_dev, p->launch_counter, 1, p->abort_stream));
    return 0;
}

extern "C" int h264e_hip_busy(h264e_hip_pool_t *p)
{
    if (!p) return 0;
    (void)hipSetDevice(p->device);
    if (p->group && hipEventQuery(p->group->ev_done) == hipErrorNotReady) return 1;
    return hipStreamQuery(p->stream) == hipErrorNotReady;
}

extern "C" int h264e_hip_read_recon(h264e_hip_pool_t *p, int chain, uint8_t *dst)
{
    if (!p || !dst || chain < 0 || chain >= p->nchains) FAIL("read_recon: bad argument");
    const size_t n = (size_t)p->G.W*p->G.H*3/2;
    const uint8_t *src = p->chains_host[chain].rec[p->ref_sel[chain]][0];
    HIPCHK(hipSetDevice(p->device));
    HIPCHK(hipMemcpy(dst, src, n, hipMemcpyDeviceToHost));
    return 0;
}

extern "C" int h264e_hip_rewind_frame(h264e_hip_pool_t *p, int chain)
{
    if (!p || chain < 0 || chain >= p->nchains) FAIL("rewind_frame: bad argument");
    p->ref_sel[chain] ^= 1;
    return 0;
}

extern "C" long h264e_hip_selftest_order(h264e_hip_pool_t *p, int jobs, int narrow, int banded, uint32_t *out, size_t cap)
{
    if (!p || jobs < 1 || jobs > p->nchains || !out) { snprintf(g_err, sizeof(g_err), "selftest_order: bad argument"); return -1; }
    const int rc = build_order(p, jobs, narrow, 0, banded ? 8 : 0);
    p->order_jobs = -1;
    if (rc) return -1;
    memcpy(out, p->order_host, sizeof(uint32_t)*(p->order_count < cap ? p->order_count : cap));
    return (long)p->order_count;
}

extern "C" long h264e_hip_selftest_merged_order(int rows, int lag, const int *member_jobs, int nmembers, uint32_t *out, size_t cap)
{
    size_t jobs = 0;
    for (int i = 0; member_jobs && i < nmembers; i++) jobs += member_jobs[i] > 0 ? (size_t)member_jobs[i] : H264E_ORDER_MAX_JOBS;
    if (rows < 1 || rows > 65536 || lag < 1 || !member_jobs || nmembers < 1 || !out || jobs >= H264E_ORDER_MAX_JOBS) { snprintf(g_err, sizeof(g_err), "selftest_merged_order: bad argument"); return -1; }
    uint32_t *ord = (uint32_t *)malloc(sizeof(uint32_t)*jobs*(size_t)rows);
    const int rc = ord ? order_by_start_step(ord, rows, lag, member_jobs, nmembers) : -1;
    if (!rc) memcpy(out, ord, sizeof(uint32_t)*(jobs*(size_t)rows < cap ? jobs*(size_t)rows : cap));
    free(ord);
    if (rc) { snprintf(g_err, sizeof(g_err), "out of host memory"); return -1; }
    return (long)(jobs*(size_t)rows);
}

extern "C" int h264e_hip_selftest_nal_escape(h264e_hip_pool_t *p, const uint8_t *src, uint32_t n, uint8_t *dst, uint32_t cap, uint32_t *out_n)
{
    if (!p || !src || !dst || !out_n) FAIL("selftest_nal_escape: bad argument");
    const size_t sb = ((size_t)n + 64 + 15) & ~(size_t)15, db = ((size_t)cap + 15) & ~(size_t)15;
    uint8_t *buf = 0;
    uint32_t res[2] = { 0, 0 };
    HIPCHK(hipSetDevice(p->device));
    if (hipMalloc((void **)&buf, sb + db + 64) != hipSuccess) FAIL("selftest_nal_escape: device allocation failed");
    hipError_t e = hipMemset(buf, 0, sb + db + 64);
    if (e == hipSuccess) e = hipMemcpy(buf, src, n, hipMemcpyHostToDevice);
    if (e == hipSuccess)
    {
        bk_launch_nal_selftest(buf + sb, cap, (const uint8_t *)buf, n, (uint32_t *)(buf + sb + db), p->stream);
        e = hipStreamSynchronize(p->stream);
    }
    if (e == hipSuccess) e = hipMemcpy(res, buf + sb + db, sizeof(res), hipMemcpyDeviceToHost);
    if (e == hipSuccess && !res[1] && res[0] <= cap) e = hipMemcpy(dst, buf + sb, res[0], hipMemcpyDeviceToHost);
    (void)hipFree(buf);
    if (e != hipSuccess) FAIL("selftest_nal_escape: %s", hipGetErrorString(e));
    *out_n = res[0];
    return res[1] ? 1 : 0;
}

extern "C" int h264e_hip_selftest_stage(h264e_hip_pool_t *p, int stage, const uint8_t *in, uint32_t nin, const int *args , uint8_t *out, uint32_t nout)
{
    if (!p || !in || !args || !out || stage < 1 || stage > 15 || nin > STAGE_IN_MAX || nout > STAGE_OUT_MAX) FAIL("selftest_stage: bad argument");
    uint8_t *buf = 0;
    HIPCHK(hipSetDevice(p->device));
    if (hipMalloc((void **)&buf, STAGE_IN_MAX + STAGE_OUT_MAX + 256) != hipSuccess) FAIL("selftest_stage: device allocation failed");
    hipError_t e = hipMemset(buf, 0, STAGE_IN_MAX + STAGE_OUT_MAX + 256);
    if (e == hipSuccess) e = hipMemcpy(buf, in, nin, hipMemcpyHostToDevice);
    if (e == hipSuccess) e = hipMemcpy(buf + STAGE_IN_MAX, args, STAGE_NARGS*sizeof(int), hipMemcpyHostToDevice);
    if (e == hipSuccess)
    {
        bk_launch_stage_selftest(stage, (const uint8_t *)buf, (const int *)(buf + STAGE_IN_MAX), buf + STAGE_IN_MAX + 128, p->stream);
        e = hipStreamSynchronize(p->stream);
    }
    if (e == hipSuccess) e = hipMemcpy(out, buf + STAGE_IN_MAX + 128, nout, hipMemcpyDeviceToHost);
    (void)hipFree(buf);
    if (e != hipSuccess) FAIL("selftest_stage: %s", hipGetErrorString(e));
    return 0;
}

#ifdef H264E_EMU
static void bk_launch_finalizer_selftest(const h264e_geom_t &G, const h264e_frame_task_t *task, int mode, const int *args, const int32_t *in, int32_t *hdr, mv32 *traj, hipStream_t)
{
    finalizer_selftest(G, *task, mode, args, in, hdr, traj);
}
#endif
extern "C" int h264e_hip_selftest_finalizer(h264e_hip_pool_t *p, int mode, const int *args , const uint8_t *in, uint32_t nin, uint8_t *out, uint32_t nout)
{
    if (!p || !args || !in || !out || mode < 1 || mode > 3) FAIL("selftest_finalizer: bad argument");
    const h264e_geom_t &G = p->G;
    const size_t A = 256;
    const auto up = [&](size_t n) { return (n + A - 1) & ~(A - 1); };
    h264e_frame_task_t T;
    h264e_chain_dev_t D;
    memset(&T, 0, sizeof(T)); memset(&D, 0, sizeof(D));
    T.active = 1;
    size_t in_bytes = 0, out_bytes = 0, row_off = 0;
    if (mode != 3)
    {
        T.nslices = args[5];
        if (T.nslices < 1 || T.nslices > H264E_MAX_SLICES || T.nslices > G.nmby || args[10] != 0 || args[10 + T.nslices] != G.nmby) FAIL("selftest_finalizer: bad slice rows");
        for (int k = 0; k <= T.nslices; k++)
        {
            if (k && args[10 + k] <= args[10 + k - 1]) FAIL("selftest_finalizer: bad slice rows");
            T.slice_row[k] = (int16_t)args[10 + k];
        }
    }
    const h264e_rowmeta_t *meta = (const h264e_rowmeta_t *)in;
    if (mode == 1)
    {
        const uint32_t cap = (uint32_t)args[8], guard = (uint32_t)args[9];
        row_off = (size_t)G.nmby*(sizeof(h264e_rowmeta_t) + sizeof(int));
        if (args[2] < 0 || args[2] > 56 || cap > (4u << 20) || guard > 4096u || (uint32_t)args[7] > (4u << 20) || nin < row_off) FAIL("selftest_finalizer: bad splice argument");
        in_bytes = row_off;
        for (int r = 0; r < G.nmby; r++)
        {
            if (meta[r].nbits > (uint32_t)G.row_words*32u || meta[r].lead_skips < 0 || meta[r].lead_skips > G.nmbx || meta[r].trail_skips < 0 || meta[r].trail_skips > G.nmbx)
                FAIL("selftest_finalizer: bad row %d", r);
            in_bytes += 4*(size_t)((meta[r].nbits + 31) >> 5);
        }
        out_bytes = FZ_HDR_INTS*4 + (size_t)cap + guard;
        T.slice_type = args[0]; T.hdr_nal = args[1]; T.hdr_nbits = args[2]; T.hdr_bits = (uint64_t)(uint32_t)args[3] | ((uint64_t)(uint32_t)args[4] << 32);
        T.arena_reset = args[6];
        D.arena_cap = cap;
    } else if (mode == 2)
    {
        const int n = args[6];
        if (n < 1 || n > FZ_NARGS - 32 || args[32 + n - 1] != G.nmby - 1) FAIL("selftest_finalizer: bad walk argument");
        for (int i = 0; i < n; i++) if (args[32 + i] < 0 || args[32 + i] >= G.nmby) FAIL("selftest_finalizer: bad walk argument");
        in_bytes = (size_t)G.nmb*(sizeof(h264e_mbrec_t) + (args[1] ? 2*sizeof(mv32) : 0));
        out_bytes = FZ_HDR_INTS*4 + (size_t)G.nmb*16;
        T.clusters[0] = args[7]; T.clusters[1] = args[8];
    } else
    {
        if (args[0] < 1 || args[0] > FZ_STEP_MAX) FAIL("selftest_finalizer: bad step argument");
        in_bytes = (size_t)args[0]*12; out_bytes = (size_t)args[0]*20;
    }
    if (nin != in_bytes || nout != out_bytes) FAIL("selftest_finalizer: operands of %u / %u bytes where mode %d takes %zu / %zu", nin, nout, mode, in_bytes, out_bytes);
    const size_t oT = 0, oD = oT + up(sizeof(T)), oA = oD + up(sizeof(D)), oIn = oA + up(FZ_NARGS*sizeof(int)), oRows = oIn + up(in_bytes);
    const size_t oF = oRows + (mode == 1 ? up((size_t)G.nmby*G.row_words*4) : 0), oOut = oF + up(sizeof(h264e_frameout_t) + 16), total = oOut + up(out_bytes);
    uint8_t *buf = 0;
    HIPCHK(hipSetDevice(p->device));
    if (hipMalloc((void **)&buf, total) != hipSuccess) FAIL("selftest_finalizer: device allocation failed");
    uint8_t *const body = buf + oOut + FZ_HDR_INTS*4;
    D.rowmeta = (h264e_rowmeta_t *)(buf + oIn); D.far_reads = (int *)(buf + oIn + (size_t)G.nmby*sizeof(h264e_rowmeta_t));
    D.rowbits = (uint32_t *)(buf + oRows);
    D.mbrec = (h264e_mbrec_t *)(buf + oIn);
    D.fout = (h264e_frameout_t *)(buf + oF); D.cursor = (uint32_t *)(buf + oF + sizeof(h264e_frameout_t));
    D.arena = body;
    T.chain_desc = (const h264e_chain_dev_t *)(buf + oD);
    if (mode == 2 && args[1]) T.clusters_per_mb = (const mv32 *)(buf + oIn + (size_t)G.nmb*sizeof(h264e_mbrec_t));
    hipError_t e = hipMemset(buf + oF, 0, oOut - oF + FZ_HDR_INTS*4);
    if (e == hipSuccess && mode != 3) e = hipMemset(body, 0xA5, out_bytes - FZ_HDR_INTS*4);
    if (e == hipSuccess) e = hipMemcpy(buf + oT, &T, sizeof(T), hipMemcpyHostToDevice);
    if (e == hipSuccess) e = hipMemcpy(buf + oD, &D, sizeof(D), hipMemcpyHostToDevice);
    if (e == hipSuccess) e = hipMemcpy(buf + oA, args, FZ_NARGS*sizeof(int), hipMemcpyHostToDevice);
    if (e == hipSuccess) e = hipMemcpy(buf + oIn, in, mode == 1 ? row_off : in_bytes, hipMemcpyHostToDevice);
    if (mode == 1)
    {
        const uint32_t cursor = (uint32_t)args[7];
        const uint8_t *src = in + row_off;
        if (e == hipSuccess) e = hipMemcpy(D.cursor, &cursor, 4, hipMemcpyHostToDevice);
        for (int r = 0; r < G.nmby && e == hipSuccess; r++)
        {
            const size_t n = 4*(size_t)((meta[r].nbits + 31) >> 5);
            if (n) e = hipMemcpy(buf + oRows + (size_t)r*G.row_words*4, src, n, hipMemcpyHostToDevice);
            src += n;
        }
    }
    if (e == hipSuccess)
    {
        int32_t *hdr = (int32_t *)(buf + oOut);
        bk_launch_finalizer_selftest(G, (const h264e_frame_task_t *)(buf + oT), mode, (const int *)(buf + oA), (const int32_t *)(buf + oIn), hdr, (mv32 *)body, p->stream);
        e = hipStreamSynchronize(p->stream);
    }
    if (e == hipSuccess) e = hipMemcpy(out, buf + oOut, out_bytes, hipMemcpyDeviceToHost);
    (void)hipFree(buf);
    if (e != hipSuccess) FAIL("selftest_finalizer: %s", hipGetErrorString(e));
    return 0;
}

extern "C" int h264e_hip_stamps_read(h264e_hip_pool_t *p, unsigned long long *dst , int reset)
{
    if (!p || !dst) FAIL("stamps_read: bad argument");
    memset(dst, 0, 48*sizeof(unsigned long long));
    for (int c = 0; c < p->nchains; c++)
    {
        unsigned long long t[48];
// ... 55 lines not shown
```

### include/h264e_hip.h

```cpp
#ifndef H264E_HIP_H
#define H264E_HIP_H
#include <stddef.h>
#include <stdint.h>
#ifdef __cplusplus
extern "C" {
#endif

typedef struct h264e_hip_pool h264e_hip_pool_t;

typedef struct
{
    int active;
    int frame_index;
    int slice_type;
    int qp;
    int speed;
    int hdr_nal;
    int hdr_nbits;
    uint64_t hdr_bits;
    int nslices;
    int32_t mv_clusters[2];
    const int32_t *mv_clusters_per_mb;
    uint16_t qdat[2][42];
    int stream_mode, slot, ref_slot, ref_in_flight;
    int first_row;
    int walk_parent;
    int walk_quiet;
    int walk_on_device;
    int32_t exact_state[2];
    int traj_from_device;
    int narrow_window;
    int denoised;
} h264e_hip_task_t;

#define H264E_HIP_MAX_SLICES 16

typedef struct
{
    uint32_t nbytes;
    int nslices;
    uint32_t slice_nbytes[H264E_HIP_MAX_SLICES];
    int all_skipped;
    int clusters_moved;
    int overflow;
    int far_reads;
    int in_device;
    int walk_status;
    int first_bad;
    int32_t state_out[2];
} h264e_hip_result_t;

typedef struct { int32_t mv0; int8_t type; uint8_t used_cand; uint8_t pad[2]; } h264e_hip_mbrec_t;

int  h264e_hip_device_count(void);
int  h264e_hip_pool_create(h264e_hip_pool_t **pool, int device, int width, int height, int nchains,
                           int frames_resident);
void h264e_hip_pool_destroy(h264e_hip_pool_t *pool);
int  h264e_hip_upload_i420(h264e_hip_pool_t *pool, int first, int nframes, const uint8_t *host_i420);
int  h264e_hip_upload_i420_async(h264e_hip_pool_t *pool, int first, int nframes, const uint8_t *pinned_i420);
int  h264e_hip_upload_wait(h264e_hip_pool_t *pool);
int  h264e_hip_upload_busy(h264e_hip_pool_t *pool);
void *h264e_hip_host_alloc(size_t bytes);
void h264e_hip_host_free(void *p);
int  h264e_hip_upload_planes(h264e_hip_pool_t *pool, int index, const uint8_t *const yuv[3], const int stride[3]);
int  h264e_hip_ingest_check(h264e_hip_pool_t *pool, int slot, int format, const void *const planes[3], const int strides[3], int pixel_bytes);
int  h264e_hip_ingest_device(h264e_hip_pool_t *pool, int slot, int format, const void *const planes[3], const int strides[3], int pixel_bytes, void *producer_stream);
int  h264e_hip_ingest_device_async(h264e_hip_pool_t *pool, int slot, int format, const void *const planes[3], const int strides[3], int pixel_bytes, void *producer_stream);
int  h264e_hip_set_color(h264e_hip_pool_t *pool, int bt709, int full_range);
int  h264e_hip_scale_check(h264e_hip_pool_t *pool, int slot, int format, const void *const planes[3], const int strides[3], const int *win);
int  h264e_hip_scale_device(h264e_hip_pool_t *pool, int slot, int format, const void *const planes[3], const int strides[3], const int *win, void *producer_stream);
int  h264e_hip_scale_device_async(h264e_hip_pool_t *pool, int slot, int format, const void *const planes[3], const int strides[3], const int *win, void *producer_stream);
int  h264e_hip_copy_timer_start(h264e_hip_pool_t *pool);
int  h264e_hip_copy_timer_stop(h264e_hip_pool_t *pool, double *ms);
void *h264e_hip_dev_malloc(int device, size_t bytes);
void h264e_hip_dev_free(void *p);
int  h264e_hip_dev_memcpy(void *dst, const void *src, size_t bytes, int to_device);
int  h264e_hip_generate_synth(h264e_hip_pool_t *pool, int first, int nframes, int t0, uint32_t seed);
int  h264e_hip_submit(h264e_hip_pool_t *pool, const h264e_hip_task_t *tasks );
int  h264e_hip_denoise_reset(h264e_hip_pool_t *pool);
int  h264e_hip_denoise_frames(h264e_hip_pool_t *pool, int first, int n, int from_zero);
int  h264e_hip_read_denoised(h264e_hip_pool_t *pool, int slot, uint8_t *dst);
int  h264e_hip_scenecut_frames(h264e_hip_pool_t *pool, int first, int n, uint32_t *hist, float *kernel_ms);
int  h264e_hip_lookahead_frames(h264e_hip_pool_t *pool, int first, int n, unsigned long long *rec, float *kernel_ms);
int  h264e_hip_lookahead_search_frames(h264e_hip_pool_t *pool, int first, int n, int range, unsigned long long *rec, float *kernel_ms);
int  h264e_hip_lookahead_read_field(h264e_hip_pool_t *pool, int frame, void *dst);
int  h264e_hip_mcdenoise_frames(h264e_hip_pool_t *pool, int first, int n, int mode, int from_zero);
int  h264e_hip_mcdenoise_read_vectors(h264e_hip_pool_t *pool, int frame, void *dst);
int  h264e_hip_mcdenoise_time(h264e_hip_pool_t *pool, double *kernel_ms, long long *frames);
typedef struct h264e_hip_group h264e_hip_group_t;
int  h264e_hip_group_create(h264e_hip_group_t **group, int device);
int  h264e_hip_group_join(h264e_hip_group_t *group, h264e_hip_pool_t *pool);
void h264e_hip_group_leave(h264e_hip_group_t *group, h264e_hip_pool_t *pool);
void h264e_hip_group_destroy(h264e_hip_group_t *group);
int  h264e_hip_sync(h264e_hip_pool_t *pool);
void h264e_hip_release(h264e_hip_pool_t *pool);
int  h264e_hip_stream_done(h264e_hip_pool_t *pool, int slot, h264e_hip_result_t *res);
const uint8_t *h264e_hip_stream_rbsp(h264e_hip_pool_t *pool, int slot);
const h264e_hip_mbrec_t *h264e_hip_stream_mbrec(h264e_hip_pool_t *pool, int slot);
int  h264e_hip_stream_fetch_traj(h264e_hip_pool_t *pool, int slot, int consumed, int32_t *dst);
int  h264e_hip_stream_fetch_nals(h264e_hip_pool_t *pool, int slot, uint8_t *dst, uint32_t nbytes);
int  h264e_hip_stream_copy_picture(h264e_hip_pool_t *pool, int from, int to);
int  h264e_hip_download_i420(h264e_hip_pool_t *pool, int first, int nframes, uint8_t *host_i420);
int  h264e_hip_stream_abort(h264e_hip_pool_t *pool);
int  h264e_hip_stream_rows_complete(h264e_hip_pool_t *pool, int slot, int *rows);
int  h264e_hip_busy(h264e_hip_pool_t *pool);
int  h264e_hip_read_recon(h264e_hip_pool_t *pool, int chain, uint8_t *dst);
int  h264e_hip_read_recon_slot(h264e_hip_pool_t *pool, int slot, uint8_t *dst);
int  h264e_hip_egress_check(h264e_hip_pool_t *pool, int slot_or_chain, int format, void *const planes[3], const int strides[3], int pixel_bytes);
int  h264e_hip_egress_slot(h264e_hip_pool_t *pool, int slot, int format, void *const planes[3], const int strides[3], int pixel_bytes, void *producer_stream);
int  h264e_hip_egress_last(h264e_hip_pool_t *pool, int chain, int format, void *const planes[3], const int strides[3], int pixel_bytes, void *producer_stream);
int  h264e_hip_egress_time(h264e_hip_pool_t *pool, int enable, double *ms, long long *calls);
int  h264e_hip_ssd_frames(h264e_hip_pool_t *pool, int n, int in0, int in_mod, int pic0, int pic_mod, uint64_t *out);
int  h264e_hip_ssim_frames(h264e_hip_pool_t *pool, int n, int in0, int in_mod, int pic0, int pic_mod, double *out);
int  h264e_hip_ssim_planes(h264e_hip_pool_t *pool, const void *a, int a_stride, const void *b, int b_stride, int w, int h, double *out);
int  h264e_hip_quality_last(h264e_hip_pool_t *pool, int chain, uint64_t ssd[3], double ssim[3]);
int  h264e_hip_quality_time(h264e_hip_pool_t *pool, int enable, double *ssd_ms, double *ssim_ms, long long *frames);
int  h264e_hip_rewind_frame(h264e_hip_pool_t *pool, int chain);
int h264e_hip_mb_counter(h264e_hip_pool_t *pool, unsigned long long *count, int reset);
void h264e_hip_profile(h264e_hip_pool_t *pool, int enable);
int  h264e_hip_profile_read(h264e_hip_pool_t *pool, double *mb_kernel_ms, double *splice_kernel_ms, int *launches);
int  h264e_hip_stamps_read(h264e_hip_pool_t *pool, unsigned long long *dst , int reset);
int  h264e_hip_timer_start(h264e_hip_pool_t *pool);
int  h264e_hip_timer_stop(h264e_hip_pool_t *pool, double *ms);
long h264e_hip_selftest_order(h264e_hip_pool_t *pool, int jobs, int narrow, int banded, uint32_t *out, size_t cap);
long h264e_hip_selftest_merged_order(int rows, int lag, const int *member_jobs, int nmembers, uint32_t *out, size_t cap);
int  h264e_hip_selftest_nal_escape(h264e_hip_pool_t *pool, const uint8_t *src, uint32_t n, uint8_t *dst, uint32_t cap, uint32_t *out_n);
int  h264e_hip_selftest_stage(h264e_hip_pool_t *pool, int stage, const uint8_t *in, uint32_t nin, const int *args , uint8_t *out, uint32_t nout);
int  h264e_hip_selftest_finalizer(h264e_hip_pool_t *pool, int mode, const int *args , const uint8_t *in, uint32_t nin, uint8_t *out, uint32_t nout);
int  h264e_hip_selftest_host_clusters_walk(int32_t state[2], const h264e_hip_mbrec_t *rec, int nmbx, int nmby, int nslices, const int32_t *used, int per_mb, int32_t *traj);
const char *h264e_hip_last_error(void);

#ifdef __cplusplus
}
#endif
#endif
```

Before: 14.99 million.

## Dispatch independent key-frame rows early in the macroblock launch order

Intra key frames that have no dependency on earlier frames get their rows ordered by row index alone, skipping the per-frame lag, so they run alongside earlier frames. This happens only when the launch does not fit in resident workgroups, and only up to a row budget. The band ordering, the kept-row bookkeeping and the keep array size are extended to match. The progress reset is also rebuilt as one host image upload instead of a memset plus per-chain copies. Risks are extra host work per launch, order rebuilds whenever the led set changes, and early key rows competing for resident slots with the frames that must finish first.

Measured after the change: 15.77 million (median of 6 runs). +5.2%, better.

```diff
diff --git a/h264-lab_amd/csrc/h264e_host.c b/h264-lab_amd/csrc/h264e_host.c
--- a/h264-lab_amd/csrc/h264e_host.c
+++ b/h264-lab_amd/csrc/h264e_host.c
@@ -899,7 +899,7 @@
 int H264E_dev_memcpy(void *dst, const void *src, size_t bytes, int to_device) { g_host_err[0] = 0; return h264e_hip_dev_memcpy(dst, src, bytes, to_device); }
 
 
-#define CLIP_KEEP_MAX 8
+#define CLIP_KEEP_MAX 96
 typedef struct { int done, ring_lo, entries; } clip_pass_t;
 struct H264E_clip_tag
 {
@@ -958,6 +958,7 @@
     double la_kernel_ms; long long la_frames;
     int la_search, la_any;
     int keep_on;
+    int key_lead;
     int nkeep;
     struct clip_keep { int frame, rows, qp, nslices, speed, denoised; } keep[CLIP_KEEP_MAX];
 };
@@ -1080,6 +1081,7 @@
     c->nframes = nframes;
     c->narrow_ok = (getenv("H264E_WIDE_WINDOW") || c->seq.nmb > 12000) ? 0 : 1;
     c->keep_on = getenv("H264E_KEEP_KEY_ROWS") ? atoi(getenv("H264E_KEEP_KEY_ROWS")) != 0 : 1;
+    c->key_lead = !c->keep_on ? 0 : getenv("H264E_KEY_LEAD") ? imax(atoi(getenv("H264E_KEY_LEAD")), 0) : -1;
     {
         const int nmb = c->seq.nmb;
         const int rows_budget = (par->slices > 1 || c->seq.nmby <= 135) ? 13000 : 6500;
@@ -1114,6 +1116,7 @@
         }
         c->ring = imax(c->launch_base + 1, c->ring/2);
     }
+    h264e_hip_set_key_lead(c->pool, c->key_lead);
     if (par->keep_records)
     {
         c->rec_store = (h264e_hip_mbrec_t **)calloc((size_t)nframes, sizeof(*c->rec_store));
@@ -1836,6 +1839,7 @@
     int qp_task[CLIP_RC_DEPTH_MAX];
     int hedge_level[CLIP_HEDGE_MAX], hedge_qp[CLIP_HEDGE_MAX];
     int kept_frames, kept_rows;
+    int led_frames, led_rows, led_last;
     int after_stop;
     double t_submit, t_first, t_last;
     double t_prev;
@@ -2087,7 +2091,7 @@
         int rows = 0;
         if (t->slice_type != SLICE_I) continue;
         if (h264e_hip_stream_rows_complete(c->pool, t->slot, &rows)) return -1;
-        if (rows <= 0) break;
+        if (rows <= 0) { if (ti > l->led_last) break; continue; }
         k->frame = l->n + ti; k->rows = rows; k->qp = t->qp; k->nslices = t->nslices; k->speed = t->speed; k->denoised = t->denoised;
         c->nkeep++;
     }
@@ -2137,8 +2141,8 @@
     const double t_end = now_ms();
     const int nvalid = l->nvalid;
     const double t_first = nvalid ? l->t_first : t_end, t_last = nvalid ? l->t_last : t_end;
-    fprintf(stderr, "clip launch %d (first row %d, %s window, %lld far reads): %d frames in flight, %d valid, next %d; first frame after %.2f ms, then %.3f ms/frame, drained %.2f ms after the last, %d key rows kept in %d frames; ended by: %s%s\n",
-            x->stats.rounds, c->tasks[0].first_row, c->tasks[0].narrow_window ? "narrow" : "wide", x->far_reads, l->F, nvalid, c->next, t_first - l->t_submit, nvalid > 1 ? (t_last - t_first)/(nvalid - 1 + (nvalid < l->F)) : 0.0, t_end - t_last, l->kept_rows, l->kept_frames,
+    fprintf(stderr, "clip launch %d (first row %d, %s window, %lld far reads): %d frames in flight, %d valid, next %d; first frame after %.2f ms, then %.3f ms/frame, drained %.2f ms after the last, %d key rows kept in %d frames, led %d key frames, %d rows; ended by: %s%s\n",
+            x->stats.rounds, c->tasks[0].first_row, c->tasks[0].narrow_window ? "narrow" : "wide", x->far_reads, l->F, nvalid, c->next, t_first - l->t_submit, nvalid > 1 ? (t_last - t_first)/(nvalid - 1 + (nvalid < l->F)) : 0.0, t_end - t_last, l->kept_rows, l->kept_frames, l->led_frames, l->led_rows,
             k_clip_ended_by[l->step], l->nh ? " (+ hedge leaves)" : "");
 }
 
@@ -2185,6 +2189,7 @@
         x.far_reads = 0;
         l.t_submit = now_ms();
         if (clip_prepass_denoise(c, l.limit) || h264e_hip_submit(c->pool, c->tasks)) return clip_end(c, &x, st, -1);
+        h264e_hip_last_lead(c->pool, &l.led_frames, &l.led_rows, &l.led_last);
         do
         {
             h264e_hip_result_t r;
diff --git a/h264-lab_amd/csrc/h264e_pool.h b/h264-lab_amd/csrc/h264e_pool.h
--- a/h264-lab_amd/csrc/h264e_pool.h
+++ b/h264-lab_amd/csrc/h264e_pool.h
@@ -164,6 +164,7 @@
     h264e_frame_task_t *tasks_dev;
     h264e_frame_task_t *tasks_host;
     int *progress_all;
+    int *progress_img;
     int *errflag;
     unsigned long long *mb_counter;
     uint32_t *order;
@@ -171,6 +172,9 @@
     uint32_t *order_host;
     int order_jobs, order_narrow, order_sliced;
     size_t order_count;
+    uint8_t *order_led, *led;
+    int key_lead;
+    int led_jobs, led_rows, led_last;
     h264e_hostdone_t *host_done;
     uint8_t **host_rbsp;
     h264e_hip_mbrec_t **host_mbrec;
@@ -196,6 +200,7 @@
     int waves;
     int test_upload_fail_at, async_uploads;
     int test_keep_rows_cap;
+    int test_lead_resident;
     double prof_mb_ms, prof_splice_ms;
     hipStream_t stream;
     hipStream_t copy_stream;
@@ -266,7 +271,7 @@
     if (p->abort_stream) (void)hipStreamSynchronize(p->abort_stream);
     device_release(p);
     host_free(p->hheap);
-    free(p->host_rbsp); free(p->host_mbrec); free(p->slot_launch); free(p->order_host); free(p->tasks_host);
+    free(p->host_rbsp); free(p->host_mbrec); free(p->slot_launch); free(p->order_host); free(p->order_led); free(p->led); free(p->progress_img); free(p->tasks_host);
     dev_free(p->heap);
     dev_free(p->den);
     dev_free(p->sc_rec);
@@ -291,7 +296,7 @@
 }
 
 #define H264E_ORDER_MAX_JOBS 65536
-static int order_by_start_step(uint32_t *out, int rows, int lag, const int *member_jobs, int nmembers)
+static int order_by_start_step(uint32_t *out, int rows, int lag, const int *member_jobs, int nmembers, const uint8_t *led)
 {
     int maxjobs = 0;
     for (int i = 0; i < nmembers; i++) if (member_jobs[i] > maxjobs) maxjobs = member_jobs[i];
@@ -299,19 +304,20 @@
     const int maxkey = lag*(maxjobs - 1) + 2*(rows - 1);
     int *start = (int *)calloc((size_t)maxkey + 2, sizeof(int));
     if (!start) return -1;
-    for (int i = 0; i < nmembers; i++) for (int j = 0; j < member_jobs[i]; j++) for (int r = 0; r < rows; r++) start[lag*j + 2*r + 1]++;
+    const auto key = [&](int job, int j, int r) { return (led && led[job] && r < rows - 1) ? 2*r : lag*j + 2*r; };
+    for (int i = 0, base = 0; i < nmembers; base += member_jobs[i], i++) for (int j = 0; j < member_jobs[i]; j++) for (int r = 0; r < rows; r++) start[key(base + j, j, r) + 1]++;
     for (int k = 0; k <= maxkey; k++) start[k + 1] += start[k];
     for (int j = 0; j < maxjobs; j++)
         for (int i = 0, base = 0; i < nmembers; base += member_jobs[i], i++)
             if (j < member_jobs[i])
-                for (int r = 0; r < rows; r++) out[start[lag*j + 2*r]++] = ((uint32_t)(base + j) << 16) | (uint32_t)r;
+                for (int r = 0; r < rows; r++) out[start[key(base + j, j, r)]++] = ((uint32_t)(base + j) << 16) | (uint32_t)r;
     free(start);
     return 0;
 }
 
 static size_t order_capacity(const h264e_geom_t &G, int jobs) { return (size_t)jobs*(size_t)(8*((G.nmby + 7)/8 + 1)); }
 
-static size_t order_into_bands(const h264e_geom_t &G, int jobs, const uint32_t *in, int total, uint32_t *out)
+static size_t order_into_bands(const h264e_geom_t &G, int jobs, const uint32_t *in, int total, uint32_t *out, const uint8_t *led)
 {
     const int bands = 8, per = (G.nmby + 7)/8 + 1;
     const size_t qlen = (size_t)per*jobs;
@@ -323,30 +329,37 @@
     for (int i = 0; i < total; i++)
     {
         const int row = (int)(in[i] & 0xffffu), x = (row >= G.nmby ? bands - 1 : imin_h(bands - 1, row*bands/G.nmby)) & 7;
-        want[8*(in[i] >> 16) + x]++;
+        if (!(led && led[in[i] >> 16] && row >= G.nmby)) want[8*(in[i] >> 16) + x]++;
     }
     for (int i = 0; i < total; i++)
     {
         const int row = (int)(in[i] & 0xffffu), jb = (int)(in[i] >> 16), x = (row >= G.nmby ? bands - 1 : imin_h(bands - 1, row*bands/G.nmby)) & 7;
-        if (row == 0) for (int y = 0; y < 8; y++) if (!want[8*jb + y]) cnt[y] += (size_t)per;
+        const int own = (led && led[jb]) ? per - 1 : per;
+        if (own < per && row >= G.nmby)
+        {
+            q[(size_t)x*qlen + cnt[x]] = in[i];
+            for (int y = 0; y < 8; y++) cnt[y]++;
+            continue;
+        }
+        if (row == 0) for (int y = 0; y < 8; y++) if (!want[8*jb + y]) cnt[y] += (size_t)own;
         q[(size_t)x*qlen + cnt[x]++] = in[i];
-        if (++fill[8*jb + x] == want[8*jb + x]) cnt[x] += (size_t)(per - want[8*jb + x]);
+        if (++fill[8*jb + x] == want[8*jb + x]) cnt[x] += (size_t)(own - want[8*jb + x]);
     }
     for (size_t k = 0; k < qlen; k++) for (int x = 0; x < 8; x++) out[n++] = q[(size_t)x*qlen + k];
     free(q); free(fill); free(want);
     return n;
 }
 
-static int build_order(h264e_hip_pool_t *p, int jobs, int narrow, int sliced, int bands)
+static int build_order(h264e_hip_pool_t *p, int jobs, int narrow, int sliced, int bands, const uint8_t *led)
 {
     const h264e_geom_t &G = p->G;
     const int rows = G.nmby + 1, total = jobs*rows, lag = narrow ? H264E_NARROW_FRAME_LAG : H264E_FRAME_LAG;
     if (bands < 0) bands = getenv("H264E_XCD_BANDS") ? atoi(getenv("H264E_XCD_BANDS")) : (G.nmb >= 30000 && !sliced ? 8 : 0);
     if (bands != 0 && bands != 8) FAIL("dispatch order: %d XCD bands (H264E_XCD_BANDS): only 0 and 8 are supported", bands);
     uint32_t *tmp = bands ? (uint32_t *)malloc(sizeof(uint32_t)*(size_t)total) : p->order_host;
-    int rc = tmp ? order_by_start_step(tmp, rows, lag, &jobs, 1) : -1;
+    int rc = tmp ? order_by_start_step(tmp, rows, lag, &jobs, 1, led) : -1;
     p->order_count = (size_t)total;
-    if (!rc && bands && !(p->order_count = order_into_bands(G, jobs, tmp, total, p->order_host))) rc = -1;
+    if (!rc && bands && !(p->order_count = order_into_bands(G, jobs, tmp, total, p->order_host, led))) rc = -1;
     if (bands) free(tmp);
     if (rc) FAIL("out of host memory");
     return 0;
@@ -374,8 +387,10 @@
     G.fz_wait_all = getenv("H264E_FZ_WAIT_ALL") ? atoi(getenv("H264E_FZ_WAIT_ALL")) : 0;
     p->test_upload_fail_at = -1;
     p->test_keep_rows_cap = -1;
+    p->test_lead_resident = -1;
     if (knobs)
     {
+        if (getenv("H264E_TEST_LEAD_RESIDENT")) p->test_lead_resident = atoi(getenv("H264E_TEST_LEAD_RESIDENT"));
         if (getenv("H264E_TEST_KEEP_ROWS_CAP")) p->test_keep_rows_cap = atoi(getenv("H264E_TEST_KEEP_ROWS_CAP"));
         if (getenv("H264E_TEST_ROW_BYTES_PER_MB")) { const int b = atoi(getenv("H264E_TEST_ROW_BYTES_PER_MB"))/4; G.row_words = G.nmbx*(b > 1 ? b : 1); }
         if (getenv("H264E_TEST_SPIN_LIMIT")) G.spin_limit = (unsigned)atol(getenv("H264E_TEST_SPIN_LIMIT"));
@@ -493,8 +508,10 @@
         FAIL("descriptor upload failed");
     }
     p->order_host = (uint32_t *)malloc(sizeof(uint32_t)*order_capacity(G, nchains));
-    if (!p->order_host) { h264e_hip_pool_destroy(p); FAIL("out of host memory"); }
+    p->order_led = (uint8_t *)calloc((size_t)nchains, 1); p->led = (uint8_t *)calloc((size_t)nchains, 1);
+    if (!p->order_host || !p->order_led || !p->led) { h264e_hip_pool_destroy(p); FAIL("out of host memory"); }
     p->order_jobs = -1;
+    p->key_lead = -1; p->led_last = -1;
     *pool = p;
     return 0;
 }
@@ -1592,6 +1609,32 @@
     if (jobs*(nmby + 1) <= H264E_RESIDENT_WG_V3) return 3;
     return 2;
 }
+static int variant_resident(int variant) { return variant == 3 ? H264E_RESIDENT_WG_V3 : variant == 4 ? 2048 : H264E_RESIDENT_WG_V2; }
+
+#define H264E_LEAD_MAX_JOBS 64
+static int lead_jobs(uint8_t *led, const int *member_jobs, int nmembers, const uint8_t *key, const int *first_row, int nmby, int tree, int all_intra,
+                     int resident, int budget, int *rows_out, int *last_out)
+{
+    int jobs = 0, maxjobs = 0, n = 0, rows = 0, last = -1, full = 0;
+    for (int i = 0; i < nmembers; i++) { jobs += member_jobs[i]; if (member_jobs[i] > maxjobs) maxjobs = member_jobs[i]; }
+    memset(led, 0, (size_t)jobs);
+    if (!tree && !all_intra && budget > 0 && (long long)jobs*(nmby + 1) > resident)
+        for (int j = 1; j < maxjobs && !full; j++)
+            for (int i = 0, base = 0; i < nmembers && !full; base += member_jobs[i], i++)
+            {
+                const int job = base + j;
+                if (j >= member_jobs[i] || !key[job]) continue;
+                const int fr = first_row[job] > 0 ? first_row[job] : 0, cost = nmby - fr;
+                if (cost <= 0) continue;
+                if (rows + cost > budget || n >= H264E_LEAD_MAX_JOBS) { full = 1; break; }
+                led[job] = 1; n++; rows += cost; last = job;
+            }
+    if (rows_out) *rows_out = rows;
+    if (last_out) *last_out = last;
+    return n;
+}
+static int lead_budget(int key_lead, int resident) { return key_lead >= 0 ? key_lead : resident/4; }
+static int lead_candidate(const h264e_frame_task_t &t) { return t.active && t.slice_type == 2 && !t.dep_progress; }
 
 static hipError_t launch_mb(const h264e_geom_t &G, int narrow, int variant, int jobs, size_t nblocks, const h264e_frame_task_t *tasks, const uint32_t *order,
                             hipEvent_t before, hipEvent_t after, hipStream_t stream)
@@ -1642,19 +1685,40 @@
     if (m.jobs >= H264E_ORDER_MAX_JOBS) return group_fail(g, "group launch: too many jobs");
     h264e_frame_task_t *th = (h264e_frame_task_t *)malloc(sizeof(h264e_frame_task_t)*(size_t)m.jobs);
     uint32_t *oh = (uint32_t *)malloc(sizeof(uint32_t)*total);
-    if (!th || !oh || order_by_start_step(oh, G.nmby + 1, narrow ? H264E_NARROW_FRAME_LAG : H264E_FRAME_LAG, jobs, n)) rc = group_fail(g, "out of host memory");
+    uint8_t *led = (uint8_t *)calloc((size_t)m.jobs, 2);
+    int *fr = (int *)malloc(sizeof(int)*(size_t)m.jobs);
+    if (!th || !oh || !led || !fr) rc = group_fail(g, "out of host memory");
     for (int i = 0, b = 0; i < n && !rc; b += jobs[i++])
     {
         h264e_hip_pool_t *p = g->member[idx[i]].pool;
         memcpy(th + b, g->member[idx[i]].tasks, sizeof(h264e_frame_task_t)*(size_t)jobs[i]);
         if (hipEventRecord(p->ev_prep, p->stream) != hipSuccess || hipStreamWaitEvent(g->stream, p->ev_prep, 0) != hipSuccess) rc = group_fail(g, "group launch: cannot order the launch behind a member's stream");
     }
+    const int variant = pick_variant(m, m.jobs, G.nmby);
+    if (!rc)
+    {
+        const int window = (12 - H264E_NARROW_FRAME_LAG)*(G.nmby + 1)/2, left = 1400 - n*(window > 0 ? window : 1);
+        uint8_t *key = led + m.jobs;
+        int key_lead = -1;
+        for (int i = 0; i < n; i++) { const int k = g->member[idx[i]].pool->key_lead; if (k >= 0 && (key_lead < 0 || k < key_lead)) key_lead = k; }
+        for (int j = 0; j < m.jobs; j++) { key[j] = (uint8_t)lead_candidate(th[j]); fr[j] = th[j].first_row; }
+        const int budget = imin_h(lead_budget(key_lead, variant_resident(variant)), left > 0 ? left : 0);
+        (void)lead_jobs(led, jobs, n, key, fr, G.nmby, m.tree, m.all_intra, variant_resident(variant), budget, 0, 0);
+        for (int i = 0, b = 0; i < n; b += jobs[i++])
+        {
+            h264e_hip_pool_t *p = g->member[idx[i]].pool;
+            p->led_jobs = p->led_rows = 0; p->led_last = -1;
+            for (int j = 0; j < jobs[i]; j++) if (led[b + j]) { p->led_jobs++; p->led_rows += G.nmby - (fr[b + j] > 0 ? fr[b + j] : 0); p->led_last = j; }
+        }
+        if (order_by_start_step(oh, G.nmby + 1, narrow ? H264E_NARROW_FRAME_LAG : H264E_FRAME_LAG, jobs, n, led)) rc = group_fail(g, "out of host memory");
+    }
+    free(led); free(fr);
     if (!rc && (hipMemcpyAsync(td, th, sizeof(h264e_frame_task_t)*(size_t)m.jobs, hipMemcpyHostToDevice, g->stream) != hipSuccess ||
                 hipMemcpyAsync(od, oh, sizeof(uint32_t)*total, hipMemcpyHostToDevice, g->stream) != hipSuccess)) rc = group_fail(g, "group launch: task upload failed");
     free(th); free(oh);
     if (!rc)
     {
-        const hipError_t le = launch_mb(G, narrow, pick_variant(m, m.jobs, G.nmby), m.jobs, total, td, od, g->ev_t0[narrow], g->ev_t1[narrow], g->stream);
+        const hipError_t le = launch_mb(G, narrow, variant, m.jobs, total, td, od, g->ev_t0[narrow], g->ev_t1[narrow], g->stream);
         if (le != hipSuccess) rc = group_fail(g, "group launch: %s", hipGetErrorString(le));
         else g->timed[narrow] = 1;
     }
@@ -1890,31 +1954,48 @@
 static int reset_progress(h264e_hip_pool_t *p, const h264e_frame_task_t *host)
 {
     const h264e_geom_t &G = p->G;
-    hipError_t e = hipMemsetAsync(p->progress_all, 0, sizeof(int)*2*(size_t)p->nchains*G.nmby, p->stream);
-    for (int c = 0; c < p->nchains && e == hipSuccess; c++)
-        if (host[c].active && host[c].first_row > 0)
-        {
-            int *done = (int *)malloc(sizeof(int)*(size_t)host[c].first_row), *progress = p->chains_host[host[c].chain].progress;
-            if (!done) { e = hipErrorOutOfMemory; break; }
-            for (int r = 0; r < host[c].first_row; r++) done[r] = G.nmbx + 1;
-            e = hipMemcpyAsync(progress, done, sizeof(int)*(size_t)host[c].first_row, hipMemcpyHostToDevice, p->stream);
-            if (e == hipSuccess) e = hipMemcpyAsync(progress + G.nmby, done, sizeof(int)*(size_t)host[c].first_row, hipMemcpyHostToDevice, p->stream);
-            free(done);
-        }
+    const size_t words = 2*(size_t)p->nchains*G.nmby;
+    int kept = 0;
+    for (int c = 0; c < p->nchains; c++) kept += host[c].active && host[c].first_row > 0;
+    hipError_t e;
+    if (!kept) e = hipMemsetAsync(p->progress_all, 0, sizeof(int)*words, p->stream);
+    else
+    {
+        if (!p->progress_img) p->progress_img = (int *)malloc(sizeof(int)*words);
+        int *img = p->progress_img;
+        if (!img) FAIL("out of host memory");
+        memset(img, 0, sizeof(int)*words);
+        for (int c = 0; c < p->nchains; c++)
+            if (host[c].active && host[c].first_row > 0)
+            {
+                int *progress = img + (size_t)host[c].chain*2*G.nmby;
+                for (int r = 0; r < host[c].first_row; r++) progress[r] = progress[G.nmby + r] = G.nmbx + 1;
+            }
+        e = hipMemcpyAsync(p->progress_all, img, sizeof(int)*words, hipMemcpyHostToDevice, p->stream);
+    }
     if (e != hipSuccess) FAIL("progress reset: %s", hipGetErrorString(e));
     return 0;
 }
 
-static int solo_launch(h264e_hip_pool_t *p, const h264e_frame_task_t *slot, const launch_shape_t &s)
-{
-    const int pe = p->ev_pending;
-    if (s.jobs != p->order_jobs || s.narrow != p->order_narrow || s.sliced != p->order_sliced)
-    {
-        if (build_order(p, s.jobs, s.narrow, s.sliced, -1)) return -1;
+static int solo_launch(h264e_hip_pool_t *p, const h264e_frame_task_t *slot, const h264e_frame_task_t *host, const launch_shape_t &s)
+{
+    const int pe = p->ev_pending, variant = pick_variant(s, s.jobs, p->G.nmby), resident = p->test_lead_resident >= 0 ? p->test_lead_resident : variant_resident(variant);
+    {
+        uint8_t *key = (uint8_t *)malloc((size_t)s.jobs);
+        int *fr = (int *)malloc(sizeof(int)*(size_t)s.jobs);
+        if (!key || !fr) { free(key); free(fr); FAIL("out of host memory"); }
+        for (int j = 0; j < s.jobs; j++) { key[j] = (uint8_t)lead_candidate(host[j]); fr[j] = host[j].first_row; }
+        p->led_jobs = lead_jobs(p->led, &s.jobs, 1, key, fr, p->G.nmby, s.tree, s.all_intra, resident, lead_budget(p->key_lead, resident), &p->led_rows, &p->led_last);
+        free(key); free(fr);
+    }
+    if (s.jobs != p->order_jobs || s.narrow != p->order_narrow || s.sliced != p->order_sliced || memcmp(p->led, p->order_led, (size_t)s.jobs))
+    {
+        if (build_order(p, s.jobs, s.narrow, s.sliced, -1, p->led_jobs ? p->led : 0)) return -1;
         HIPCHK(hipMemcpyAsync(p->order, p->order_host, sizeof(uint32_t)*p->order_count, hipMemcpyHostToDevice, p->stream));
         p->order_jobs = s.jobs; p->order_narrow = s.narrow; p->order_sliced = s.sliced;
-    }
-    const hipError_t e = launch_mb(p->G, s.narrow, pick_variant(s, s.jobs, p->G.nmby), s.jobs, p->order_count, slot, p->order,
+        memcpy(p->order_led, p->led, (size_t)s.jobs);
+    }
+    const hipError_t e = launch_mb(p->G, s.narrow, variant, s.jobs, p->order_count, slot, p->order,
                                    p->profile ? p->ev[pe][0] : 0, p->profile ? p->ev[pe][1] : 0, p->stream);
     if (e != hipSuccess) FAIL("macroblock kernel launch: %s", hipGetErrorString(e));
     if (p->profile)
@@ -1945,7 +2026,15 @@
     const hipError_t e = hipMemcpyAsync(slot, host, sizeof(h264e_frame_task_t)*(size_t)p->nchains, hipMemcpyHostToDevice, p->stream);
     if (e != hipSuccess) FAIL("task upload: %s", hipGetErrorString(e));
     if (reset_progress(p, host)) return -1;
-    return p->group ? group_submit(p, host, s) : solo_launch(p, slot, s);
+    return p->group ? group_submit(p, host, s) : solo_launch(p, slot, host, s);
+}
+
+extern "C" void h264e_hip_set_key_lead(h264e_hip_pool_t *p, int budget) { if (p) p->key_lead = budget < 0 ? -1 : budget; }
+extern "C" void h264e_hip_last_lead(h264e_hip_pool_t *p, int *jobs, int *rows, int *last)
+{
+    if (jobs) *jobs = p ? p->led_jobs : 0;
+    if (rows) *rows = p ? p->led_rows : 0;
+    if (last) *last = p ? p->led_last : -1;
 }
 
 
@@ -2075,7 +2164,7 @@
 extern "C" long h264e_hip_selftest_order(h264e_hip_pool_t *p, int jobs, int narrow, int banded, uint32_t *out, size_t cap)
 {
     if (!p || jobs < 1 || jobs > p->nchains || !out) { snprintf(g_err, sizeof(g_err), "selftest_order: bad argument"); return -1; }
-    const int rc = build_order(p, jobs, narrow, 0, banded ? 8 : 0);
+    const int rc = build_order(p, jobs, narrow, 0, banded ? 8 : 0, 0);
     p->order_jobs = -1;
     if (rc) return -1;
     memcpy(out, p->order_host, sizeof(uint32_t)*(p->order_count < cap ? p->order_count : cap));
@@ -2088,11 +2177,41 @@
     for (int i = 0; member_jobs && i < nmembers; i++) jobs += member_jobs[i] > 0 ? (size_t)member_jobs[i] : H264E_ORDER_MAX_JOBS;
     if (rows < 1 || rows > 65536 || lag < 1 || !member_jobs || nmembers < 1 || !out || jobs >= H264E_ORDER_MAX_JOBS) { snprintf(g_err, sizeof(g_err), "selftest_merged_order: bad argument"); return -1; }
     uint32_t *ord = (uint32_t *)malloc(sizeof(uint32_t)*jobs*(size_t)rows);
-    const int rc = ord ? order_by_start_step(ord, rows, lag, member_jobs, nmembers) : -1;
+    const int rc = ord ? order_by_start_step(ord, rows, lag, member_jobs, nmembers, 0) : -1;
     if (!rc) memcpy(out, ord, sizeof(uint32_t)*(jobs*(size_t)rows < cap ? jobs*(size_t)rows : cap));
     free(ord);
     if (rc) { snprintf(g_err, sizeof(g_err), "out of host memory"); return -1; }
     return (long)(jobs*(size_t)rows);
+}
+
+extern "C" long h264e_hip_selftest_lead_order(int nmby, int lag, const int *member_jobs, int nmembers, const uint8_t *key, const int *first_row,
+                                              int tree, int all_intra, int resident, int budget, int banded, uint32_t *out, size_t cap, uint8_t *led_out)
+{
+    size_t jobs = 0;
+    for (int i = 0; member_jobs && i < nmembers; i++) jobs += member_jobs[i] > 0 ? (size_t)member_jobs[i] : H264E_ORDER_MAX_JOBS;
+    if (nmby < 1 || nmby >= 65535 || lag < 1 || !member_jobs || nmembers < 1 || !key || !first_row || !out || jobs >= H264E_ORDER_MAX_JOBS || (banded && nmembers != 1))
+    { snprintf(g_err, sizeof(g_err), "selftest_lead_order: bad argument"); return -1; }
+    const size_t rows = (size_t)nmby + 1, total = jobs*rows;
+    h264e_geom_t G;
+    memset(&G, 0, sizeof(G));
+    G.nmby = nmby;
+    const size_t room = banded ? order_capacity(G, (int)jobs) : total;
+    uint32_t *ord = (uint32_t *)malloc(sizeof(uint32_t)*total), *res = banded ? (uint32_t *)malloc(sizeof(uint32_t)*room) : ord;
+    uint8_t *led = (uint8_t *)malloc(jobs);
+    size_t n = total;
+    int rc = (ord && res && led) ? 0 : -1;
+    if (!rc)
+    {
+        const int nled = lead_jobs(led, member_jobs, nmembers, key, first_row, nmby, tree, all_intra, resident, budget, 0, 0);
+        rc = order_by_start_step(ord, (int)rows, lag, member_jobs, nmembers, nled ? led : 0);
+        if (!rc && banded && !(n = order_into_bands(G, (int)jobs, ord, (int)total, res, nled ? led : 0))) rc = -1;
+    }
+    if (!rc) memcpy(out, res, sizeof(uint32_t)*(n < cap ? n : cap));
+    if (!rc && led_out) memcpy(led_out, led, jobs);
+    if (banded) free(res);
+    free(ord); free(led);
+    if (rc) { snprintf(g_err, sizeof(g_err), "out of host memory"); return -1; }
+    return (long)n;
 }
 
 extern "C" int h264e_hip_selftest_nal_escape(h264e_hip_pool_t *p, const uint8_t *src, uint32_t n, uint8_t *dst, uint32_t cap, uint32_t *out_n)
diff --git a/include/h264e_hip.h b/include/h264e_hip.h
--- a/include/h264e_hip.h
+++ b/include/h264e_hip.h
@@ -103,6 +103,8 @@
 int  h264e_hip_download_i420(h264e_hip_pool_t *pool, int first, int nframes, uint8_t *host_i420);
 int  h264e_hip_stream_abort(h264e_hip_pool_t *pool);
 int  h264e_hip_stream_rows_complete(h264e_hip_pool_t *pool, int slot, int *rows);
+void h264e_hip_set_key_lead(h264e_hip_pool_t *pool, int budget);
+void h264e_hip_last_lead(h264e_hip_pool_t *pool, int *jobs, int *rows, int *last);
 int  h264e_hip_busy(h264e_hip_pool_t *pool);
 int  h264e_hip_read_recon(h264e_hip_pool_t *pool, int chain, uint8_t *dst);
 int  h264e_hip_read_recon_slot(h264e_hip_pool_t *pool, int slot, uint8_t *dst);
@@ -124,6 +126,8 @@
 int  h264e_hip_timer_stop(h264e_hip_pool_t *pool, double *ms);
 long h264e_hip_selftest_order(h264e_hip_pool_t *pool, int jobs, int narrow, int banded, uint32_t *out, size_t cap);
 long h264e_hip_selftest_merged_order(int rows, int lag, const int *member_jobs, int nmembers, uint32_t *out, size_t cap);
+long h264e_hip_selftest_lead_order(int nmby, int lag, const int *member_jobs, int nmembers, const uint8_t *key, const int *first_row,
+                                   int tree, int all_intra, int resident, int budget, int banded, uint32_t *out, size_t cap, uint8_t *led_out);
 int  h264e_hip_selftest_nal_escape(h264e_hip_pool_t *pool, const uint8_t *src, uint32_t n, uint8_t *dst, uint32_t cap, uint32_t *out_n);
 int  h264e_hip_selftest_stage(h264e_hip_pool_t *pool, int stage, const uint8_t *in, uint32_t nin, const int *args , uint8_t *out, uint32_t nout);
 int  h264e_hip_selftest_finalizer(h264e_hip_pool_t *pool, int mode, const int *args , const uint8_t *in, uint32_t nin, uint8_t *out, uint32_t nout);
```
